# ygjwd12345/UCD

Measured on NVIDIA B200. Metric: ucd_loss_fwd_bwd_pixel_pairs_per_s, higher is better.
Workload: dtype bf16 operands / f32 accumulate (contrastive); f32 (CE, KD, upsample)

## Files before the change

### include/ucd_b200.h

```cpp
#ifndef UCD_B200_H
#define UCD_B200_H

#include <stddef.h>
#include <stdint.h>

#ifdef __cplusplus
extern "C" {
#endif

#define UCD_OK 0
#define UCD_EINVAL (-1)
#define UCD_ECUDA (-2)
#define UCD_ENOSUP (-3)

#define UCD_REDUCTION_NONE 0
#define UCD_REDUCTION_MEAN 1
#define UCD_REDUCTION_SUM 2

#define UCD_FEAT_DIM 256
#define UCD_TILE 128

int ucd_version(void);
const char* ucd_last_error(void);
int ucd_device_ok(void);

int ucd_unce_fwd(const float* x, int64_t* y, float* loss_px, float* lse_all, float* lse_old,
                 float* stats , float* scratch ,
                 int B, int C, int old_cl, int64_t HW, int ignore_index, void* stream);
int ucd_unce_bwd(const float* x, const int64_t* y, const float* lse_all,
                 const float* bkg_gap ,
                 const float* g_px, const float* g_scalar, float g_mul, const float* stats,
                 int mean_over_valid, float* dx, int accumulate, int B, int C, int old_cl, int64_t HW,
                 int ignore_index, void* stream);

int ucd_unkd_fwd(const float* x, const float* t, const float* mask, float alpha, float* out_px,
                 float* stats, float* lse3, float* scratch, int B, int C, int C_old, int64_t HW,
                 void* stream);
int ucd_unkd_bwd(const float* x, const float* t, const float* mask, float alpha, const float* lse3,
                 const float* g_px, const float* g_scalar, float g_mul, float* dx, int accumulate, int B, int C,
                 int C_old, int64_t HW, void* stream);
size_t ucd_reduce_scratch_floats(void);

int ucd_kd_fwd(const float* x, const float* t, const float* mask, float alpha, float* out_px, float* stats,
               float* lse3, float* scratch, int B, int C, int C_old, int64_t HW, int variant, float stats_scale,
               void* stream);
int ucd_kd_bwd(const float* x, const float* t, const float* mask, float alpha, const float* lse3,
               const float* g_px, const float* g_scalar, float g_mul, float* dx, int accumulate, int B, int C,
               int C_old, int64_t HW, int variant, void* stream);
int ucd_unce_unkd_bwd(const float* x, const int64_t* y, const float* lse_all, const float* bkg_gap ,
                      const float* ce_g_px, const float* ce_g_scalar, float ce_g_mul, const float* ce_stats,
                      int mean_over_valid, int old_cl, int ignore_index, const float* t, const float* mask,
                      float alpha, const float* lse3, const float* kd_g_px, const float* kd_g_scalar, float kd_g_mul,
                      int kd_variant, float* dx, int accumulate, int B, int C, int C_old, int64_t HW, void* stream);
int ucd_bkg_mask(const float* t_old, const int64_t* labels, float* mask, int B, int C_old, int64_t HW,
                 int old_cl, void* stream);

int ucd_upsample_bilinear_fwd(const float* in, float* out, int64_t planes, int h, int w, int H, int W,
                              void* stream);
int ucd_upsample_bilinear_bwd(const float* gout, float* gin, int64_t planes, int h, int w, int H, int W,
                              void* stream);

size_t ucd_seg_fused_workspace_floats(int B, int C, int C_old, int h, int w, int H, int W);
int ucd_seg_fused_fwd(const float* lr, const float* lr_old, int64_t* labels, float* g_ce, float* g_kd,
                      float* sums, float* workspace, size_t workspace_floats, int B, int C, int C_old, int h,
                      int w, int H, int W, int old_cl, int ignore_index, float alpha, int need_grad,
                      void* stream);

int64_t ucd_con_max_tiles(int64_t n_px);
int ucd_con_prob_kpad(int C_old);
int ucd_con_num_bins(int max_label, int C_old);
int64_t ucd_con_px_meta_ints(int64_t n_px);
int64_t ucd_con_blk_meta_ints(int64_t n_px, int nb);
int ucd_con_prep_labels(const int64_t* labels, const float* l_po, int B, int C_old, int h, int w,
                        int H, int W, int max_label, int32_t* px_meta, int32_t* blk_meta, int32_t* counts,
                        int32_t* counts_host ,
                        void* stream);
int ucd_con_prep_pack(const float* f_n, const float* f_o, const float* l_po, const int32_t* px_meta,
                      int32_t* blk_meta, const int32_t* counts, int B, int C_old, int h, int w, int max_label,
                      float* anchor_f32, float* contrast_f32, void* la, void* lc,
                      int label_bytes ,
                      void* feat_tiles, void* prob_tiles, int32_t* lab_tiles, int32_t* tile_range,
                      int32_t* row_range , int32_t* row_ref, float* inv_norm,
                      int64_t max_tiles, void* stream);
int ucd_con_prep_bwd(const float* g_anchor, const float* anchor_f32, const float* inv_norm,
                     const int32_t* px_meta, const int32_t* blk_meta, float* df_n, int B, int h, int w,
                     void* stream);
int ucd_con_prep_pack_bf16(const void* f_n, const void* f_o, const float* l_po, const int32_t* px_meta,
                           int32_t* blk_meta, const int32_t* counts, int B, int C_old, int h, int w, int max_label,
                           float* anchor_f32, float* contrast_f32, void* la, void* lc, int label_bytes,
                           void* feat_tiles, void* prob_tiles, int32_t* lab_tiles, int32_t* tile_range,
                           int32_t* row_range, int32_t* row_ref, float* inv_norm, int64_t max_tiles, void* stream);
int ucd_con_prep_bwd_bf16(const float* g_anchor, const float* anchor_f32, const float* inv_norm,
                          const int32_t* px_meta, const int32_t* blk_meta, void* df_n, int B, int h, int w,
                          void* stream);
int ucd_con_tile_ranges(const int32_t* lab_tiles, int64_t n_tiles, const int32_t* n_limit, int32_t* tile_range,
                        void* stream);
int ucd_con_pack_rows(const float* rows, const int32_t* labels, int64_t n, void* feat_tiles,
                      int32_t* lab_tiles, int64_t max_tiles, void* stream);

int ucd_rows_normalize_fwd(const float* f, float* rows, float* inv_norm, int B, int h, int w, void* stream);
int ucd_rows_normalize_bwd(const float* g_rows, const float* rows, const float* inv_norm, float* df, int B, int h,
                           int w, void* stream);

size_t ucd_con_workspace_bytes(int64_t max_row_tiles, int64_t max_col_tiles, int64_t plan_row_tiles,
                               int64_t local_col_tiles );
int ucd_con_fwd(const void* feat_tiles, const void* prob_tiles, const int32_t* lab_tiles,
                const int32_t* chunk_counts, int n_chunks, int64_t chunk_tiles, int64_t chunk_stride_bytes,
                int local_chunk, int part, const void* row_feat_tiles,
                const void* row_prob_tiles, const int32_t* row_lab_tiles, const int32_t* n_rows,
                const int32_t* tile_range, const int32_t* row_range, int64_t self_tile0, const int32_t* min_new, int p_mode, int kpad, const float* dense_p,
                int64_t ldp, float inv_temperature, int need_grad, float* out, float* grad_unit,
                void* workspace, size_t workspace_bytes, int64_t max_row_tiles, int64_t plan_row_tiles,
                void* stream);
size_t ucd_selfcon_workspace_bytes(int64_t tiles );
int ucd_selfcon_fwd(const void* feat_tiles, const int32_t* lab_tiles, const int32_t* tile_range, const int32_t* counts,
                    const int32_t* n_rows, int64_t n, int64_t n_anchor, int mode, float inv_temperature, float kappa,
                    int need_grad, float* out, float* grad_unit, void* workspace, size_t workspace_bytes, void* stream);
int ucd_con_bwd(const float* grad_unit, const float* out, const float* g_scalar, float g_mul,
                const int32_t* n_rows, const int32_t* row_ref, float* d_anchor, int64_t max_rows, void* stream);

#ifdef __cplusplus
}
#endif
#endif
```

### ucd_b200/_lib.py

```python
import ctypes
import os
from ctypes import c_float, c_int, c_int64, c_size_t, c_void_p

_HERE = os.path.dirname(os.path.abspath(__file__))
LIB_PATH = os.path.join(_HERE, "libucd_b200.so")

_lib = None

P = c_void_p
_PROTOS = {
    "ucd_version": (c_int, []),
    "ucd_last_error": (ctypes.c_char_p, []),
    "ucd_device_ok": (c_int, []),
    "ucd_reduce_scratch_floats": (c_size_t, []),
    "ucd_unce_fwd": (c_int, [P, P, P, P, P, P, P, c_int, c_int, c_int, c_int64, c_int, P]),
    "ucd_unce_bwd": (c_int, [P, P, P, P, P, P, c_float, P, c_int, P, c_int, c_int, c_int, c_int, c_int64, c_int, P]),
    "ucd_unkd_fwd": (c_int, [P, P, P, c_float, P, P, P, P, c_int, c_int, c_int, c_int64, P]),
    "ucd_unkd_bwd": (c_int, [P, P, P, c_float, P, P, P, c_float, P, c_int, c_int, c_int, c_int, c_int64, P]),
    "ucd_kd_fwd": (c_int, [P, P, P, c_float, P, P, P, P, c_int, c_int, c_int, c_int64, c_int, c_float, P]),
    "ucd_kd_bwd": (c_int, [P, P, P, c_float, P, P, P, c_float, P, c_int, c_int, c_int, c_int, c_int64, c_int, P]),
    "ucd_unce_unkd_bwd": (c_int, [P, P, P, P, P, P, c_float, P, c_int, c_int, c_int, P, P, c_float, P, P, P, c_float, c_int,
                                  P, c_int, c_int, c_int, c_int, c_int64, P]),
    "ucd_bkg_mask": (c_int, [P, P, P, c_int, c_int, c_int64, c_int, P]),
    "ucd_upsample_bilinear_fwd": (c_int, [P, P, c_int64, c_int, c_int, c_int, c_int, P]),
    "ucd_upsample_bilinear_bwd": (c_int, [P, P, c_int64, c_int, c_int, c_int, c_int, P]),
    "ucd_seg_fused_workspace_floats": (c_size_t, [c_int, c_int, c_int, c_int, c_int, c_int, c_int]),
    "ucd_seg_fused_fwd": (c_int, [P, P, P, P, P, P, P, c_size_t, c_int, c_int, c_int, c_int, c_int, c_int, c_int,
                                  c_int, c_int, c_float, c_int, P]),
    "ucd_con_max_tiles": (c_int64, [c_int64]),
    "ucd_con_prob_kpad": (c_int, [c_int]),
    "ucd_con_num_bins": (c_int, [c_int, c_int]),
    "ucd_con_px_meta_ints": (c_int64, [c_int64]),
    "ucd_con_blk_meta_ints": (c_int64, [c_int64, c_int]),
    "ucd_con_prep_labels": (c_int, [P, P, c_int, c_int, c_int, c_int, c_int, c_int, c_int, P, P, P, P, P]),
    "ucd_con_prep_pack": (c_int, [P, P, P, P, P, P, c_int, c_int, c_int, c_int, c_int, P, P, P, P, c_int, P, P, P, P,
                                  P, P, P, c_int64, P]),
    "ucd_con_prep_bwd": (c_int, [P, P, P, P, P, P, c_int, c_int, c_int, P]),
    "ucd_con_prep_pack_bf16": (c_int, [P, P, P, P, P, P, c_int, c_int, c_int, c_int, c_int, P, P, P, P, c_int, P, P, P,
                                       P, P, P, P, c_int64, P]),
    "ucd_con_prep_bwd_bf16": (c_int, [P, P, P, P, P, P, c_int, c_int, c_int, P]),
    "ucd_rows_normalize_fwd": (c_int, [P, P, P, c_int, c_int, c_int, P]),
    "ucd_rows_normalize_bwd": (c_int, [P, P, P, P, c_int, c_int, c_int, P]),
    "ucd_con_tile_ranges": (c_int, [P, c_int64, P, P, P]),
    "ucd_con_pack_rows": (c_int, [P, P, c_int64, P, P, c_int64, P]),
    "ucd_con_workspace_bytes": (c_size_t, [c_int64, c_int64, c_int64, c_int64]),
    "ucd_con_fwd": (c_int, [P, P, P, P, c_int, c_int64, c_int64, c_int, c_int, P, P, P, P, P, P, c_int64, P, c_int, c_int,
                            P, c_int64, c_float, c_int, P, P, P, c_size_t, c_int64, c_int64, P]),
    "ucd_con_bwd": (c_int, [P, P, P, c_float, P, P, P, c_int64, P]),
    "ucd_selfcon_workspace_bytes": (c_size_t, [c_int64]),
    "ucd_selfcon_fwd": (c_int, [P, P, P, P, P, c_int64, c_int64, c_int, c_float, c_float, c_int, P, P, P, c_size_t, P]),
}
EXPORTED = tuple(_PROTOS)
_DEBUG_PROTOS = {
    "ucd_con_debug_trace": (c_int, [P]),
    "ucd_con_debug_splits": (c_int, [c_int64, c_int64]),
    "ucd_selftest_umma": (c_int, [c_int, ctypes.POINTER(c_float)]),
    "ucd_selftest_mma_rate": (c_int, [c_int, c_int, ctypes.POINTER(c_float)]),
    "ucd_selftest_mma_mix": (c_int, [c_int] * 8 + [ctypes.POINTER(c_float)]),
    "ucd_selftest_pipe_rate": (c_int, [c_int, c_int, c_int, ctypes.POINTER(c_float)]),
    "ucd_selftest_read_probe": (c_int, [P, ctypes.c_longlong, c_int, c_int, c_int, c_int, ctypes.POINTER(c_float)]),
}
DEBUG_EXPORTED = tuple(_DEBUG_PROTOS)
DEBUG_LIB_PATH = os.path.join(_HERE, "libucd_b200_debug.so")
_debug = None


def lib():
    global _lib
    if _lib is None:
        if not os.path.exists(LIB_PATH):
            raise RuntimeError(
                "ucd_b200: %s is missing - build it with `python -m ucd_b200.build` "
                "(there is no CPU or PyTorch fallback for this path)" % LIB_PATH)
        h = ctypes.CDLL(LIB_PATH)
        for name, (res, args) in _PROTOS.items():
            fn = getattr(h, name)
            fn.restype = res
            fn.argtypes = args
        _lib = h
    return _lib


def debug_lib(as_product=False):
    global _debug, _lib
    if _debug is None:
        if not os.path.exists(DEBUG_LIB_PATH):
            raise RuntimeError("ucd_b200: %s is missing - build it with `python -m ucd_b200.build --debug`" % DEBUG_LIB_PATH)
        h = ctypes.CDLL(DEBUG_LIB_PATH)
        for name, (res, args) in list(_PROTOS.items()) + list(_DEBUG_PROTOS.items()):
            fn = getattr(h, name)
            fn.restype = res
            fn.argtypes = args
        _debug = h
    if as_product:
        _lib = _debug
    return _debug


class _NvtxProxy:

    def __init__(self, handle):
        self._h = handle

    def __getattr__(self, name):
        fn = getattr(self._h, name)
        if not name.startswith("ucd_") or name in ("ucd_last_error", "ucd_version", "ucd_device_ok"):
            return fn
        import torch

        def wrapped(*args):
            torch.cuda.nvtx.range_push(name)
            try:
                return fn(*args)
            finally:
                torch.cuda.nvtx.range_pop()
        return wrapped


def enable_nvtx(on=True):
    global _lib
    h = lib()
    if on and not isinstance(h, _NvtxProxy):
        _lib = _NvtxProxy(h)
    elif not on and isinstance(h, _NvtxProxy):
        _lib = h._h


def check(rc, what=""):
    if rc != 0:
        msg = lib().ucd_last_error().decode("utf-8", "replace")
        raise RuntimeError("ucd_b200 %s failed (code %d): %s" % (what, rc, msg))


def ptr(t):
    if t is None:
        return None
    return c_void_p(t) if isinstance(t, int) else c_void_p(t.data_ptr())


_raw_stream = None


def cur_stream():
    global _raw_stream
    import torch
    if _raw_stream is None:
        get_raw = getattr(torch._C, "_cuda_getCurrentRawStream", None)
        get_dev = getattr(torch._C, "_cuda_getDevice", None)
        if get_raw is not None and get_dev is not None:
            _raw_stream = lambda: get_raw(get_dev())
        else:
            _raw_stream = lambda: torch.cuda.current_stream().cuda_stream
    return c_void_p(_raw_stream())
```

### ucd_b200/csrc/ce_kd.cu

```cuda
#include "common.cuh"

namespace ucd {

constexpr int kStreamThreads = 256;
constexpr int kStreamMaxBlocks = kNumSMs * 8;
constexpr int kScratchFloats = 4 * kStreamMaxBlocks + 64;

template <int VEC>
struct Vec;
template <>
struct Vec<4> {
  static __device__ __forceinline__ void load(const float* p, float (&v)[4]) {
    float4 t = ldg_stream4(p);
    v[0] = t.x, v[1] = t.y, v[2] = t.z, v[3] = t.w;
  }
  static __device__ __forceinline__ void load_cached(const float* p, float (&v)[4]) {
    float4 t = *reinterpret_cast<const float4*>(p);
    v[0] = t.x, v[1] = t.y, v[2] = t.z, v[3] = t.w;
  }
  static __device__ __forceinline__ void store(float* p, const float (&v)[4]) {
    *reinterpret_cast<float4*>(p) = make_float4(v[0], v[1], v[2], v[3]);
  }
  static __device__ __forceinline__ void store_stream(float* p, const float (&v)[4]) {
    stg_stream4(p, make_float4(v[0], v[1], v[2], v[3]));
  }
};
template <>
struct Vec<1> {
  static __device__ __forceinline__ void load(const float* p, float (&v)[1]) { v[0] = ldg_stream1(p); }
  static __device__ __forceinline__ void load_cached(const float* p, float (&v)[1]) { v[0] = *p; }
  static __device__ __forceinline__ void store(float* p, const float (&v)[1]) { *p = v[0]; }
  static __device__ __forceinline__ void store_stream(float* p, const float (&v)[1]) { stg_stream1(p, v[0]); }
};

template <int VEC, bool ACC>
__device__ __forceinline__ void store_dx(float* p, float (&o)[VEC]) {
  if (ACC) {
    float old[VEC];
    Vec<VEC>::load(p, old);
#pragma unroll
    for (int i = 0; i < VEC; ++i) o[i] += old[i];
  }
  Vec<VEC>::store_stream(p, o);
}

__global__ void reduce_partials_kernel(const float* __restrict__ part, int nblk, int nk, float* __restrict__ out,
                                       float scale) {
  __shared__ float red[32];
  for (int k = 0; k < nk; ++k) {
    float acc = 0.f;
    for (int i = threadIdx.x; i < nblk; i += blockDim.x) acc += part[(size_t)k * nblk + i];
    float r = block_sum(acc, red);
    if (threadIdx.x == 0) out[k] = r * scale;
  }
}

constexpr float kNegBig = -3.0e38f;
constexpr int kLseChunk = 8;

template <int VEC, bool PICK>
__device__ __forceinline__ void lse_chunks(const float* __restrict__ xp, long long HW, int c0, int c1,
                                           const long long (&lab)[VEC], float (&m)[VEC], float (&s)[VEC],
                                           float (&picked)[VEC]) {
  for (int c = c0; c < c1; c += kLseChunk) {
    float v[kLseChunk][VEC];
#pragma unroll
    for (int k = 0; k < kLseChunk; ++k) {
      if (c + k < c1) {
        Vec<VEC>::load(xp + (long long)(c + k) * HW, v[k]);
      } else {
#pragma unroll
        for (int i = 0; i < VEC; ++i) v[k][i] = kNegBig;
      }
    }
#pragma unroll
    for (int i = 0; i < VEC; ++i) {
      float cm = v[0][i];
#pragma unroll
      for (int k = 1; k < kLseChunk; ++k) cm = fmaxf(cm, v[k][i]);
      const float nm = fmaxf(m[i], cm * kLog2e);
      float acc = s[i] * ex2f(m[i] - nm);
#pragma unroll
      for (int k = 0; k < kLseChunk; ++k) {
        acc += ex2f(fmaf(v[k][i], kLog2e, -nm));
        if (PICK) picked[i] = (lab[i] == c + k) ? v[k][i] : picked[i];
      }
      m[i] = nm;
      s[i] = acc;
    }
  }
}

template <int VEC>
__device__ __forceinline__ void lse_chunk4(const float (&v)[4][VEC], float (&m)[VEC], float (&s)[VEC]) {
#pragma unroll
  for (int i = 0; i < VEC; ++i) {
    const float cm = fmaxf(fmaxf(v[0][i], v[1][i]), fmaxf(v[2][i], v[3][i]));
    const float nm = fmaxf(m[i], cm * kLog2e);
    float acc = s[i] * ex2f(m[i] - nm);
#pragma unroll
    for (int k = 0; k < 4; ++k) acc += ex2f(fmaf(v[k][i], kLog2e, -nm));
    m[i] = nm;
    s[i] = acc;
  }
}

template <int VEC>
__device__ __forceinline__ void lse_planes(const float*& xc, long long HW, int n, float (&m)[VEC], float (&s)[VEC]) {
  int c = 0;
  for (; c + 4 <= n; c += 4) {
    float v[4][VEC];
    Vec<VEC>::load(xc, v[0]);
    Vec<VEC>::load(xc + HW, v[1]);
    Vec<VEC>::load(xc + 2 * HW, v[2]);
    Vec<VEC>::load(xc + 3 * HW, v[3]);
    xc += 4 * HW;
    lse_chunk4<VEC>(v, m, s);
  }
  if (c < n) {
    float v[4][VEC];
#pragma unroll
    for (int k = 0; k < 4; ++k) {
      if (c + k < n) {
        Vec<VEC>::load(xc + k * HW, v[k]);
      } else {
#pragma unroll
        for (int i = 0; i < VEC; ++i) v[k][i] = kNegBig;
      }
    }
    xc += (long long)(n - c) * HW;
    lse_chunk4<VEC>(v, m, s);
  }
}

__device__ __forceinline__ void group_to_bp(long long g, long long gpi, bool small, int vec, long long& b, long long& p) {
  if (small) {
    const unsigned bb = (unsigned)g / (unsigned)gpi;
    b = bb;
    p = (long long)((unsigned)g - bb * (unsigned)gpi) * vec;
  } else {
    b = g / gpi;
    p = (g - b * gpi) * vec;
  }
}

template <int VEC>
__global__ void __launch_bounds__(kStreamThreads, VEC == 4 ? 4 : 2)
unce_fwd_kernel(const float* __restrict__ x, long long* __restrict__ y, float* __restrict__ loss_px,
                float* __restrict__ lse_all_out, float* __restrict__ lse_old_out, float* __restrict__ part,
                int B, int C, int old_cl, long long HW, int ignore_index) {
  const long long gpi = HW / VEC;
  const long long n_groups = gpi * B;
  const bool small = n_groups < (1ll << 31) && gpi < (1ll << 31);
  const int oc = old_cl < C ? (old_cl > 0 ? old_cl : 0) : C;
  float loss_acc = 0.f, valid_acc = 0.f;
  for (long long g = (long long)blockIdx.x * blockDim.x + threadIdx.x; g < n_groups;
       g += (long long)gridDim.x * blockDim.x) {
    long long b, p;
    group_to_bp(g, gpi, small, VEC, b, p);
    const float* xp = x + (b * C) * HW + p;
    long long* yp = y + b * HW + p;
    long long yl[VEC];
    if (VEC == 4) {
      const longlong2 t0 = *reinterpret_cast<const longlong2*>(yp), t1 = *reinterpret_cast<const longlong2*>(yp + 2);
      yl[0] = t0.x, yl[1] = t0.y, yl[2 % VEC] = t1.x, yl[3 % VEC] = t1.y;
    } else {
#pragma unroll
      for (int i = 0; i < VEC; ++i) yl[i] = yp[i];
    }
    int lab[VEC];
    float picked[VEC];
#pragma unroll
    for (int i = 0; i < VEC; ++i) {
      long long t = yl[i];
      if (t < old_cl) {
        if (t != 0) yp[i] = 0;
        t = 0;
      }
      lab[i] = (t < 0 || t > 0x7fffffffLL) ? -1 : (int)t;
      picked[i] = (lab[i] >= 0 && lab[i] < C) ? __ldg(xp + (long long)lab[i] * HW + i) : 0.f;
    }
    float m[VEC], s[VEC], lse_old2[VEC];
#pragma unroll
    for (int i = 0; i < VEC; ++i) m[i] = kNegBig, s[i] = 0.f;
    const float* xc = xp;
    lse_planes<VEC>(xc, HW, oc, m, s);
#pragma unroll
    for (int i = 0; i < VEC; ++i) lse_old2[i] = m[i] + lg2f(s[i]);
    lse_planes<VEC>(xc, HW, C - oc, m, s);
    float out[VEC], la[VEC], lo[VEC];
#pragma unroll
    for (int i = 0; i < VEC; ++i) {
      const float lse2 = m[i] + lg2f(s[i]);
      la[i] = lse2 * kLn2;
      lo[i] = lse_old2[i] * kLn2;
      const bool ign = lab[i] == ignore_index;
      float l = (lab[i] == 0 && old_cl > 0) ? (la[i] - lo[i]) : (la[i] - picked[i]);
      if (ign || lab[i] < 0 || lab[i] >= C) l = 0.f;
      out[i] = l;
      loss_acc += l;
      valid_acc += ign ? 0.f : 1.f;
    }
    Vec<VEC>::store(loss_px + b * HW + p, out);
    Vec<VEC>::store(lse_all_out + b * HW + p, la);
    if (lse_old_out != nullptr) Vec<VEC>::store(lse_old_out + b * HW + p, lo);
  }
  if (part != nullptr) {
    __shared__ float red[32];
    float r0 = block_sum(loss_acc, red);
    float r1 = block_sum(valid_acc, red);
    if (threadIdx.x == 0) {
      part[blockIdx.x] = r0;
      part[gridDim.x + blockIdx.x] = r1;
    }
  }
}

template <int VEC, bool ACC>
__global__ void __launch_bounds__(kStreamThreads)
unce_bwd_kernel(const float* __restrict__ x, const long long* __restrict__ y, const float* __restrict__ lse_all,
                const float* __restrict__ bkg_gap, const float* __restrict__ g_px,
                const float* __restrict__ g_scalar, float g_mul, const float* __restrict__ stats,
                int mean_over_valid, float* __restrict__ dx, int B, int C, int old_cl, long long HW,
                int ignore_index) {
  const long long gpi = HW / VEC;
  const long long n_groups = gpi * B;
  float gs = 0.f;
  if (g_px == nullptr) {
    gs = g_scalar[0] * g_mul;
    if (mean_over_valid) gs = gs / stats[1];
  }
  for (long long g = (long long)blockIdx.x * blockDim.x + threadIdx.x; g < n_groups;
       g += (long long)gridDim.x * blockDim.x) {
    const long long b = g / gpi, p = (g - b * gpi) * VEC;
    const float* xp = x + (b * C) * HW + p;
    float* dp = dx + (b * C) * HW + p;
    const long long* yp = y + b * HW + p;
    float la2[VEC], up[VEC], fold[VEC];
    int lab[VEC];
    {
      float la[VEC], lo[VEC], gp[VEC];
      Vec<VEC>::load_cached(lse_all + b * HW + p, la);
      Vec<VEC>::load_cached(bkg_gap + b * HW + p, lo);
      if (g_px != nullptr) Vec<VEC>::load_cached(g_px + b * HW + p, gp);
#pragma unroll
      for (int i = 0; i < VEC; ++i) {
        long long t = yp[i];
        if (t < old_cl) t = 0;
        const bool dead = (t == ignore_index) || t < 0 || t >= C;
        lab[i] = dead ? -1 : (int)t;
        up[i] = dead ? 0.f : (g_px != nullptr ? gp[i] : gs);
        la2[i] = la[i] * kLog2e;
        fold[i] = ex2f(lo[i] * kLog2e);
      }
    }
#pragma unroll 4
    for (int c = 0; c < C; ++c) {
      float v[VEC], o[VEC];
      Vec<VEC>::load(xp + (long long)c * HW, v);
#pragma unroll
      for (int i = 0; i < VEC; ++i) {
        const float pr = ex2f(fmaf(v[i], kLog2e, -la2[i]));
        float sub;
        if (lab[i] == 0 && old_cl > 0)
          sub = (c < old_cl) ? pr * fold[i] : 0.f;
        else
          sub = (c == lab[i]) ? 1.f : 0.f;
        o[i] = up[i] * (pr - sub);
      }
      store_dx<VEC, ACC>(dp + (long long)c * HW, o);
    }
  }
}

template <int VEC, bool TAIL>
__device__ __forceinline__ void unkd_old_chunk(const float (&v)[4][VEC], const float (&u)[4][VEC], int nv, bool skip0,
                                               float a2, float (&m)[VEC], float (&s)[VEC], float (&mt)[VEC],
                                               float (&st)[VEC], float (&wx)[VEC]) {
#pragma unroll
  for (int i = 0; i < VEC; ++i) {
    float cm = v[0][i], ct = u[0][i] * a2;
#pragma unroll
    for (int k = 1; k < 4; ++k) {
      const bool live = !TAIL || k < nv;
      cm = live ? fmaxf(cm, v[k][i]) : cm;
      ct = live ? fmaxf(ct, u[k][i] * a2) : ct;
    }
    const float nm = fmaxf(m[i], cm * kLog2e), nt = fmaxf(mt[i], ct);
    float acc = s[i] * ex2f(m[i] - nm);
    const float rs = ex2f(mt[i] - nt);
    float tacc = st[i] * rs, wacc = wx[i] * rs;
#pragma unroll
    for (int k = 0; k < 4; ++k) {
      const bool live = !TAIL || k < nv;
      const float ex = ex2f(fmaf(v[k][i], kLog2e, -nm));
      const float et = ex2f(fmaf(u[k][i], a2, -nt));
      acc += live ? ex : 0.f;
      tacc += live ? et : 0.f;
      const float w = (live && !(k == 0 && skip0)) ? et : 0.f;
      wacc = fmaf(w, v[k][i], wacc);
    }
    m[i] = nm, s[i] = acc, mt[i] = nt, st[i] = tacc, wx[i] = wacc;
  }
}

template <int VEC>
__global__ void __launch_bounds__(kStreamThreads, VEC == 4 ? 3 : 2)
unkd_fwd_kernel(const float* __restrict__ x, const float* __restrict__ t, const float* __restrict__ mask,
                float alpha, float* __restrict__ out_px, float* __restrict__ lse3, float* __restrict__ part,
                int B, int C, int Cs, int C_old, int mask_zero, long long HW) {
  const long long gpi = HW / VEC;
  const long long n_groups = gpi * B;
  const bool small = n_groups < (1ll << 31) && gpi < (1ll << 31);
  const long long plane = (long long)B * HW;
  const float a2 = alpha * kLog2e;
  const float inv_cold = 1.f / (float)C_old;
  float acc = 0.f;
  for (long long g = (long long)blockIdx.x * blockDim.x + threadIdx.x; g < n_groups;
       g += (long long)gridDim.x * blockDim.x) {
    long long b, p;
    group_to_bp(g, gpi, small, VEC, b, p);
    const float* xp = x + (b * Cs) * HW + p;
    const float* xc = xp;
    const float* tc = t + (b * C_old) * HW + p;
    float m[VEC], s[VEC], mt[VEC], st[VEC], wx[VEC], x0[VEC], t0[VEC];
#pragma unroll
    for (int i = 0; i < VEC; ++i) m[i] = mt[i] = kNegBig, s[i] = st[i] = wx[i] = 0.f;
    int c = 0;
    for (; c + 4 <= C_old; c += 4) {
      float v[4][VEC], u[4][VEC];
#pragma unroll
      for (int k = 0; k < 4; ++k) {
        Vec<VEC>::load(xc + k * HW, v[k]);
        Vec<VEC>::load(tc + k * HW, u[k]);
      }
      xc += 4 * HW, tc += 4 * HW;
      if (c == 0) {
#pragma unroll
        for (int i = 0; i < VEC; ++i) x0[i] = v[0][i], t0[i] = u[0][i] * a2;
      }
      unkd_old_chunk<VEC, false>(v, u, 4, c == 0, a2, m, s, mt, st, wx);
    }
    if (c < C_old) {
      const int nv = C_old - c;
      float v[4][VEC], u[4][VEC];
#pragma unroll
      for (int k = 0; k < 4; ++k) {
        if (k < nv) {
          Vec<VEC>::load(xc + k * HW, v[k]);
          Vec<VEC>::load(tc + k * HW, u[k]);
        } else {
#pragma unroll
          for (int i = 0; i < VEC; ++i) v[k][i] = 0.f, u[k][i] = 0.f;
        }
      }
      if (c == 0) {
#pragma unroll
        for (int i = 0; i < VEC; ++i) x0[i] = v[0][i], t0[i] = u[0][i] * a2;
      }
      unkd_old_chunk<VEC, true>(v, u, nv, c == 0, a2, m, s, mt, st, wx);
    }
    float mn[VEC], sn[VEC];
#pragma unroll
    for (int i = 0; i < VEC; ++i) mn[i] = kNegBig, sn[i] = 0.f;
    xc = xp + (long long)C_old * HW;
    lse_planes<VEC>(xc, HW, C - C_old, mn, sn);
    float o[VEC], l_all[VEC], l_bkg[VEC], l_t[VEC];
    float mk[VEC];
    if (mask != nullptr) Vec<VEC>::load_cached(mask + b * HW + p, mk);
#pragma unroll
    for (int i = 0; i < VEC; ++i) {
      const float ma = fmaxf(m[i], mn[i]);
      const float lse2 = ma + lg2f(fmaf(s[i], ex2f(m[i] - ma), sn[i] * ex2f(mn[i] - ma)));
      const float x02 = x0[i] * kLog2e;
      const float mb = fmaxf(x02, mn[i]);
      const float lseb2 = mb + lg2f(fmaf(sn[i], ex2f(mn[i] - mb), ex2f(x02 - mb)));
      const float lset2 = mt[i] + lg2f(st[i]);
      l_all[i] = lse2 * kLn2;
      l_bkg[i] = lseb2 * kLn2;
      l_t[i] = lset2 * kLn2;
      const float q0 = ex2f(t0[i] - lset2);
      const float dot = wx[i] / st[i];
      float l = (q0 * (l_bkg[i] - l_all[i]) + dot - (1.f - q0) * l_all[i]) * inv_cold;
      if (mask != nullptr) l *= mask_zero ? (mk[i] == 0.f ? 1.f : 0.f) : mk[i];
      o[i] = -l;
      acc += l;
    }
    if (out_px != nullptr) Vec<VEC>::store(out_px + b * HW + p, o);
    Vec<VEC>::store(lse3 + b * HW + p, l_all);
    Vec<VEC>::store(lse3 + plane + b * HW + p, l_bkg);
    Vec<VEC>::store(lse3 + 2 * plane + b * HW + p, l_t);
  }
  __shared__ float red[32];
  float r = block_sum(acc, red);
  if (threadIdx.x == 0) part[blockIdx.x] = r;
}

template <int VEC, bool ACC>
__global__ void __launch_bounds__(kStreamThreads)
unkd_bwd_kernel(const float* __restrict__ x, const float* __restrict__ t, const float* __restrict__ mask,
                float alpha, const float* __restrict__ lse3, const float* __restrict__ g_px,
                const float* __restrict__ g_scalar, float g_mul, float* __restrict__ dx, int B, int C, int Cs,
                int C_old, int mask_zero, long long HW) {
  const long long gpi = HW / VEC;
  const long long n_groups = gpi * B;
  const long long plane = (long long)B * HW;
  const float a2 = alpha * kLog2e;
  const float inv_cold = 1.f / (float)C_old;
  const float gs = (g_px == nullptr) ? g_scalar[0] * g_mul : 0.f;
  for (long long g = (long long)blockIdx.x * blockDim.x + threadIdx.x; g < n_groups;
       g += (long long)gridDim.x * blockDim.x) {
    const long long b = g / gpi, p = (g - b * gpi) * VEC;
    const float* xp = x + (b * Cs) * HW + p;
    const float* tp = t + (b * C_old) * HW + p;
    float* dp = dx + (b * Cs) * HW + p;
    float la2[VEC], lt2[VEC], up[VEC], fb[VEC];
    {
      float la[VEC], lb[VEC], lt[VEC], gp[VEC], mk[VEC], u0[VEC];
      Vec<VEC>::load_cached(lse3 + b * HW + p, la);
      Vec<VEC>::load_cached(lse3 + plane + b * HW + p, lb);
      Vec<VEC>::load_cached(lse3 + 2 * plane + b * HW + p, lt);
      Vec<VEC>::load_cached(tp, u0);
      if (g_px != nullptr) Vec<VEC>::load_cached(g_px + b * HW + p, gp);
      if (mask != nullptr) Vec<VEC>::load_cached(mask + b * HW + p, mk);
#pragma unroll
      for (int i = 0; i < VEC; ++i) {
        la2[i] = la[i] * kLog2e;
        lt2[i] = lt[i] * kLog2e;
        float u = (g_px != nullptr ? gp[i] : gs) * inv_cold;
        if (mask != nullptr) u *= mask_zero ? (mk[i] == 0.f ? 1.f : 0.f) : mk[i];
        up[i] = u;
        const float q0 = ex2f(fmaf(u0[i], a2, -lt2[i]));
        fb[i] = q0 * ex2f((la[i] - lb[i]) * kLog2e);
      }
    }
    {
      float v[VEC], o[VEC];
      Vec<VEC>::load(xp, v);
#pragma unroll
      for (int i = 0; i < VEC; ++i) {
        const float pr = ex2f(fmaf(v[i], kLog2e, -la2[i]));
        o[i] = up[i] * (pr - pr * fb[i]);
      }
      store_dx<VEC, ACC>(dp, o);
    }
#pragma unroll 4
    for (int c = 1; c < C_old; ++c) {
      float v[VEC], u[VEC], o[VEC];
      Vec<VEC>::load(xp + (long long)c * HW, v);
      Vec<VEC>::load(tp + (long long)c * HW, u);
#pragma unroll
      for (int i = 0; i < VEC; ++i) {
        const float pr = ex2f(fmaf(v[i], kLog2e, -la2[i]));
        const float q = ex2f(fmaf(u[i], a2, -lt2[i]));
        o[i] = up[i] * (pr - q);
      }
      store_dx<VEC, ACC>(dp + (long long)c * HW, o);
    }
#pragma unroll 4
    for (int c = C_old; c < C; ++c) {
      float v[VEC], o[VEC];
      Vec<VEC>::load(xp + (long long)c * HW, v);
#pragma unroll
      for (int i = 0; i < VEC; ++i) {
        const float pr = ex2f(fmaf(v[i], kLog2e, -la2[i]));
        o[i] = up[i] * (pr - pr * fb[i]);
      }
      store_dx<VEC, ACC>(dp + (long long)c * HW, o);
    }
    if (!ACC)
      for (int c = C; c < Cs; ++c) {
        float o[VEC];
#pragma unroll
        for (int i = 0; i < VEC; ++i) o[i] = 0.f;
        Vec<VEC>::store_stream(dp + (long long)c * HW, o);
      }
  }
}

template <int VEC, bool ACC>
__global__ void __launch_bounds__(kStreamThreads)
unce_unkd_bwd_kernel(const float* __restrict__ x, const long long* __restrict__ y, const float* __restrict__ lse_all,
                     const float* __restrict__ bkg_gap, const float* __restrict__ ce_g_px,
                     const float* __restrict__ ce_g_scalar, float ce_g_mul, const float* __restrict__ ce_stats,
                     int mean_over_valid, int old_cl, int ignore_index, const float* __restrict__ t,
                     const float* __restrict__ mask, float alpha, const float* __restrict__ lse3,
                     const float* __restrict__ kd_g_px, const float* __restrict__ kd_g_scalar, float kd_g_mul,
                     int mask_zero, float* __restrict__ dx, int B, int C, int C_old, long long HW) {
  const long long gpi = HW / VEC;
  const long long n_groups = gpi * B;
  const long long plane = (long long)B * HW;
  const float a2 = alpha * kLog2e;
  const float inv_cold = 1.f / (float)C_old;
  float gs_ce = 0.f;
  if (ce_g_px == nullptr) {
    gs_ce = ce_g_scalar[0] * ce_g_mul;
    if (mean_over_valid) gs_ce = gs_ce / ce_stats[1];
  }
  const float gs_kd = (kd_g_px == nullptr) ? kd_g_scalar[0] * kd_g_mul : 0.f;
  for (long long g = (long long)blockIdx.x * blockDim.x + threadIdx.x; g < n_groups;
       g += (long long)gridDim.x * blockDim.x) {
    const long long b = g / gpi, p = (g - b * gpi) * VEC;
    const float* xp = x + (b * C) * HW + p;
    const float* tp = t + (b * C_old) * HW + p;
    float* dp = dx + (b * C) * HW + p;
    const long long* yp = y + b * HW + p;
    float la2[VEC], lt2[VEC], uce[VEC], ukd[VEC], fold[VEC], fb[VEC];
    int lab[VEC];
    {
      float la[VEC], lo[VEC], lb[VEC], lt[VEC], gp[VEC], gk[VEC], mk[VEC], u0[VEC];
      Vec<VEC>::load_cached(lse_all + b * HW + p, la);
      Vec<VEC>::load_cached(bkg_gap + b * HW + p, lo);
      Vec<VEC>::load_cached(lse3 + plane + b * HW + p, lb);
      Vec<VEC>::load_cached(lse3 + 2 * plane + b * HW + p, lt);
      Vec<VEC>::load_cached(tp, u0);
      if (ce_g_px != nullptr) Vec<VEC>::load_cached(ce_g_px + b * HW + p, gp);
      if (kd_g_px != nullptr) Vec<VEC>::load_cached(kd_g_px + b * HW + p, gk);
      if (mask != nullptr) Vec<VEC>::load_cached(mask + b * HW + p, mk);
#pragma unroll
      for (int i = 0; i < VEC; ++i) {
        long long tt = yp[i];
        if (tt < old_cl) tt = 0;
        const bool dead = (tt == ignore_index) || tt < 0 || tt >= C;
        lab[i] = dead ? -1 : (int)tt;
        uce[i] = dead ? 0.f : (ce_g_px != nullptr ? gp[i] : gs_ce);
        la2[i] = la[i] * kLog2e;
        lt2[i] = lt[i] * kLog2e;
        fold[i] = ex2f(lo[i] * kLog2e);
        float u = (kd_g_px != nullptr ? gk[i] : gs_kd) * inv_cold;
        if (mask != nullptr) u *= mask_zero ? (mk[i] == 0.f ? 1.f : 0.f) : mk[i];
        ukd[i] = u;
        const float q0 = ex2f(fmaf(u0[i], a2, -lt2[i]));
        fb[i] = q0 * ex2f((la[i] - lb[i]) * kLog2e);
      }
    }
#pragma unroll 4
    for (int c = 0; c < C; ++c) {
      float v[VEC], u[VEC], o[VEC];
      Vec<VEC>::load(xp + (long long)c * HW, v);
      const bool old_fg = c >= 1 && c < C_old;
      if (old_fg) Vec<VEC>::load(tp + (long long)c * HW, u);
#pragma unroll
      for (int i = 0; i < VEC; ++i) {
        const float pr = ex2f(fmaf(v[i], kLog2e, -la2[i]));
        float sub_ce;
        if (lab[i] == 0 && old_cl > 0)
          sub_ce = (c < old_cl) ? pr * fold[i] : 0.f;
        else
          sub_ce = (c == lab[i]) ? 1.f : 0.f;
        const float sub_kd = old_fg ? ex2f(fmaf(u[i], a2, -lt2[i])) : pr * fb[i];
        o[i] = fmaf(uce[i], pr - sub_ce, ukd[i] * (pr - sub_kd));
      }
      store_dx<VEC, ACC>(dp + (long long)c * HW, o);
    }
  }
}

__global__ void __launch_bounds__(kStreamThreads)
bkg_mask_kernel(const float* __restrict__ t, const long long* __restrict__ y, float* __restrict__ mask, int B,
                int C_old, long long HW, int old_cl) {
  const long long n = (long long)B * HW;
  for (long long g = (long long)blockIdx.x * blockDim.x + threadIdx.x; g < n; g += (long long)gridDim.x * blockDim.x) {
    const long long b = g / HW, p = g - b * HW;
    const float* tp = t + (b * C_old) * HW + p;
    const float t0 = ldg_stream1(tp);
    const bool t0_nan = t0 != t0;
    bool bkg = true;
    for (int c = 1; c < C_old; ++c) {
      const float v = ldg_stream1(tp + (long long)c * HW);
      if (!t0_nan && (v > t0 || v != v)) bkg = false;
    }
    mask[g] = (bkg || y[g] > old_cl) ? 1.f : 0.f;
  }
}

static int stream_grid(long long n_groups) {
  long long blocks = (n_groups + kStreamThreads - 1) / kStreamThreads;
  if (blocks > kStreamMaxBlocks) blocks = kStreamMaxBlocks;
  if (blocks < 1) blocks = 1;
  return (int)blocks;
}

static bool can_vec4(long long HW, std::initializer_list<const void*> ptrs) {
  if (HW % 4 != 0) return false;
  for (const void* p : ptrs)
    if (p != nullptr && !aligned16(p)) return false;
  return true;
}

}

using namespace ucd;

extern "C" size_t ucd_reduce_scratch_floats(void) { return (size_t)kScratchFloats; }

extern "C" int ucd_unce_fwd(const float* x, int64_t* y, float* loss_px, float* lse_all, float* lse_old,
                            float* stats, float* scratch, int B, int C, int old_cl, int64_t HW,
                            int ignore_index, void* stream) {
  UCD_CHECK_ARG(x && y && loss_px && lse_all, "ucd_unce_fwd: null pointer");
  UCD_CHECK_ARG(B > 0 && C > 0 && HW > 0, "ucd_unce_fwd: bad shape B=%d C=%d HW=%lld", B, C, (long long)HW);
  UCD_CHECK_ARG(old_cl >= 0 && old_cl <= C, "ucd_unce_fwd: old_cl=%d outside [0,%d]", old_cl, C);
  UCD_CHECK_ARG(stats == nullptr || scratch != nullptr, "ucd_unce_fwd: stats requested without scratch");
  cudaStream_t st = (cudaStream_t)stream;
  float* part = stats ? scratch : nullptr;
  const bool v4 = can_vec4(HW, {x, loss_px, lse_all, lse_old}) && aligned16(y);
  const int grid = stream_grid((long long)B * HW / (v4 ? 4 : 1));
  if (v4)
    unce_fwd_kernel<4><<<grid, kStreamThreads, 0, st>>>(x, (long long*)y, loss_px, lse_all, lse_old, part, B, C,
                                                        old_cl, HW, ignore_index);
  else
    unce_fwd_kernel<1><<<grid, kStreamThreads, 0, st>>>(x, (long long*)y, loss_px, lse_all, lse_old, part, B, C,
                                                        old_cl, HW, ignore_index);
  UCD_CHECK_LAUNCH("unce_fwd_kernel");
  if (stats) {
    reduce_partials_kernel<<<1, 256, 0, st>>>(part, grid, 2, stats, 1.f);
    UCD_CHECK_LAUNCH("reduce_partials_kernel");
  }
  return UCD_OK;
}

extern "C" int ucd_unce_bwd(const float* x, const int64_t* y, const float* lse_all, const float* bkg_gap,
                            const float* g_px, const float* g_scalar, float g_mul, const float* stats,
                            int mean_over_valid, float* dx, int accumulate, int B, int C, int old_cl, int64_t HW,
                            int ignore_index, void* stream) {
  UCD_CHECK_ARG(x && y && lse_all && bkg_gap && dx, "ucd_unce_bwd: null pointer");
  UCD_CHECK_ARG(g_px || g_scalar, "ucd_unce_bwd: need g_px or g_scalar");
  UCD_CHECK_ARG(!mean_over_valid || stats, "ucd_unce_bwd: mean_over_valid needs stats");
  UCD_CHECK_ARG(B > 0 && C > 0 && HW > 0, "ucd_unce_bwd: bad shape");
  cudaStream_t st = (cudaStream_t)stream;
  const bool v4 = can_vec4(HW, {x, lse_all, bkg_gap, g_px, dx}) && aligned16(y);
  const int grid = stream_grid((long long)B * HW / (v4 ? 4 : 1));
  auto kern = v4 ? (accumulate ? unce_bwd_kernel<4, true> : unce_bwd_kernel<4, false>)
                 : (accumulate ? unce_bwd_kernel<1, true> : unce_bwd_kernel<1, false>);
  kern<<<grid, kStreamThreads, 0, st>>>(x, (const long long*)y, lse_all, bkg_gap, g_px, g_scalar, g_mul, stats,
                                        mean_over_valid, dx, B, C, old_cl, HW, ignore_index);
  UCD_CHECK_LAUNCH("unce_bwd_kernel");
  return UCD_OK;
}

static int kd_fwd_impl(const float* x, const float* t, const float* mask, float alpha, float* out_px, float* stats,
                       float* lse3, float* scratch, int B, int C, int C_old, int64_t HW, int variant, float stats_scale,
                       void* stream) {
  UCD_CHECK_ARG(x && t && stats && lse3 && scratch, "ucd_kd_fwd: null pointer");
  UCD_CHECK_ARG(B > 0 && HW > 0 && C_old >= 1 && C >= C_old, "ucd_kd_fwd: bad shape C=%d C_old=%d", C, C_old);
  UCD_CHECK_ARG(variant >= 0 && variant <= 2, "ucd_kd_fwd: bad variant %d", variant);
  cudaStream_t st = (cudaStream_t)stream;
  const int Cu = variant == 1 ? C_old : C, mz = variant == 2 ? 1 : 0;
  const bool v4 = can_vec4(HW, {x, t, mask, out_px, lse3}) && ((long long)B * HW) % 4 == 0;
  const int grid = stream_grid((long long)B * HW / (v4 ? 4 : 1));
  if (v4)
    unkd_fwd_kernel<4><<<grid, kStreamThreads, 0, st>>>(x, t, mask, alpha, out_px, lse3, scratch, B, Cu, C, C_old, mz, HW);
  else
    unkd_fwd_kernel<1><<<grid, kStreamThreads, 0, st>>>(x, t, mask, alpha, out_px, lse3, scratch, B, Cu, C, C_old, mz, HW);
  UCD_CHECK_LAUNCH("unkd_fwd_kernel");
  reduce_partials_kernel<<<1, 256, 0, st>>>(scratch, grid, 1, stats, stats_scale);
  UCD_CHECK_LAUNCH("reduce_partials_kernel");
  return UCD_OK;
}

static int kd_bwd_impl(const float* x, const float* t, const float* mask, float alpha, const float* lse3,
                       const float* g_px, const float* g_scalar, float g_mul, float* dx, int accumulate, int B, int C,
                       int C_old, int64_t HW, int variant, void* stream) {
  UCD_CHECK_ARG(x && t && lse3 && dx, "ucd_kd_bwd: null pointer");
  UCD_CHECK_ARG(g_px || g_scalar, "ucd_kd_bwd: need g_px or g_scalar");
  UCD_CHECK_ARG(B > 0 && HW > 0 && C_old >= 1 && C >= C_old, "ucd_kd_bwd: bad shape");
  UCD_CHECK_ARG(variant >= 0 && variant <= 2, "ucd_kd_bwd: bad variant %d", variant);
  cudaStream_t st = (cudaStream_t)stream;
  const int Cu = variant == 1 ? C_old : C, mz = variant == 2 ? 1 : 0;
  const bool v4 = can_vec4(HW, {x, t, mask, g_px, lse3, dx}) && ((long long)B * HW) % 4 == 0;
  const int grid = stream_grid((long long)B * HW / (v4 ? 4 : 1));
  auto kern = v4 ? (accumulate ? unkd_bwd_kernel<4, true> : unkd_bwd_kernel<4, false>)
                 : (accumulate ? unkd_bwd_kernel<1, true> : unkd_bwd_kernel<1, false>);
  kern<<<grid, kStreamThreads, 0, st>>>(x, t, mask, alpha, lse3, g_px, g_scalar, g_mul, dx, B, Cu, C, C_old, mz, HW);
  UCD_CHECK_LAUNCH("unkd_bwd_kernel");
  return UCD_OK;
}

extern "C" int ucd_unkd_fwd(const float* x, const float* t, const float* mask, float alpha, float* out_px,
                            float* stats, float* lse3, float* scratch, int B, int C, int C_old, int64_t HW,
                            void* stream) {
  return kd_fwd_impl(x, t, mask, alpha, out_px, stats, lse3, scratch, B, C, C_old, HW, 0, 1.f, stream);
}

extern "C" int ucd_unkd_bwd(const float* x, const float* t, const float* mask, float alpha, const float* lse3,
                            const float* g_px, const float* g_scalar, float g_mul, float* dx, int accumulate, int B,
                            int C, int C_old, int64_t HW, void* stream) {
  return kd_bwd_impl(x, t, mask, alpha, lse3, g_px, g_scalar, g_mul, dx, accumulate, B, C, C_old, HW, 0, stream);
}

extern "C" int ucd_kd_fwd(const float* x, const float* t, const float* mask, float alpha, float* out_px,
                          float* stats, float* lse3, float* scratch, int B, int C, int C_old, int64_t HW,
                          int variant, float stats_scale, void* stream) {
  return kd_fwd_impl(x, t, mask, alpha, out_px, stats, lse3, scratch, B, C, C_old, HW, variant, stats_scale, stream);
}

extern "C" int ucd_kd_bwd(const float* x, const float* t, const float* mask, float alpha, const float* lse3,
                          const float* g_px, const float* g_scalar, float g_mul, float* dx, int accumulate, int B,
                          int C, int C_old, int64_t HW, int variant, void* stream) {
  return kd_bwd_impl(x, t, mask, alpha, lse3, g_px, g_scalar, g_mul, dx, accumulate, B, C, C_old, HW, variant, stream);
}

extern "C" int ucd_bkg_mask(const float* t_old, const int64_t* labels, float* mask, int B, int C_old, int64_t HW,
                            int old_cl, void* stream) {
  UCD_CHECK_ARG(t_old && labels && mask, "ucd_bkg_mask: null pointer");
  UCD_CHECK_ARG(B > 0 && C_old >= 1 && HW > 0, "ucd_bkg_mask: bad shape");
  bkg_mask_kernel<<<stream_grid((long long)B * HW), kStreamThreads, 0, (cudaStream_t)stream>>>(
      t_old, (const long long*)labels, mask, B, C_old, HW, old_cl);
  UCD_CHECK_LAUNCH("bkg_mask_kernel");
  return UCD_OK;
}

extern "C" int ucd_unce_unkd_bwd(const float* x, const int64_t* y, const float* lse_all, const float* bkg_gap,
                                 const float* ce_g_px, const float* ce_g_scalar, float ce_g_mul, const float* ce_stats,
                                 int mean_over_valid, int old_cl, int ignore_index, const float* t, const float* mask,
                                 float alpha, const float* lse3, const float* kd_g_px, const float* kd_g_scalar,
                                 float kd_g_mul, int kd_variant, float* dx, int accumulate, int B, int C, int C_old,
                                 int64_t HW, void* stream) {
  UCD_CHECK_ARG(x && y && lse_all && bkg_gap && t && lse3 && dx, "ucd_unce_unkd_bwd: null pointer");
  UCD_CHECK_ARG((ce_g_px || ce_g_scalar) && (kd_g_px || kd_g_scalar), "ucd_unce_unkd_bwd: need g_px or g_scalar for both terms");
  UCD_CHECK_ARG(!mean_over_valid || ce_stats, "ucd_unce_unkd_bwd: mean_over_valid needs stats");
  UCD_CHECK_ARG(B > 0 && HW > 0 && C_old >= 1 && C >= C_old, "ucd_unce_unkd_bwd: bad shape");
  UCD_CHECK_ARG(kd_variant == 0 || kd_variant == 2, "ucd_unce_unkd_bwd: KD variant must be 0 (unbiased) or 2 (masked)");
  cudaStream_t st = (cudaStream_t)stream;
  const bool v4 = can_vec4(HW, {x, lse_all, bkg_gap, ce_g_px, t, mask, lse3, kd_g_px, dx}) && aligned16(y) &&
                  ((long long)B * HW) % 4 == 0;
  const int grid = stream_grid((long long)B * HW / (v4 ? 4 : 1));
  auto kern = v4 ? (accumulate ? unce_unkd_bwd_kernel<4, true> : unce_unkd_bwd_kernel<4, false>)
                 : (accumulate ? unce_unkd_bwd_kernel<1, true> : unce_unkd_bwd_kernel<1, false>);
  kern<<<grid, kStreamThreads, 0, st>>>(x, (const long long*)y, lse_all, bkg_gap, ce_g_px, ce_g_scalar, ce_g_mul,
                                        ce_stats, mean_over_valid, old_cl, ignore_index, t, mask, alpha, lse3, kd_g_px,
                                        kd_g_scalar, kd_g_mul, kd_variant == 2 ? 1 : 0, dx, B, C, C_old, HW);
  UCD_CHECK_LAUNCH("unce_unkd_bwd_kernel");
  return UCD_OK;
}
```

### ucd_b200/csrc/upsample.cu

```cuda
#include "common.cuh"

#include <stdlib.h>

namespace ucd {

constexpr int kUpThreads = 256;

template <int VEC>
__global__ void __launch_bounds__(kUpThreads)
upsample_fwd_kernel(const float* __restrict__ in, float* __restrict__ out, long long planes, int h, int w, int H,
                    int W, float scale_h, float scale_w, int planes_per_block) {
  const int wv = (W + VEC - 1) / VEC;
  const long long idx = (long long)blockIdx.x * blockDim.x + threadIdx.x;
  if (idx >= (long long)H * wv) return;
  const int Y = (int)(idx / wv);
  const int X = (int)(idx - (long long)Y * wv) * VEC;
  const Tap ty = bilinear_tap(Y, scale_h, h, H);
  int x0[VEC], x1[VEC];
  float wx0[VEC], wx1[VEC];
  const bool small_out = H + W <= 128;
  bool uniform = true;
#pragma unroll
  for (int i = 0; i < VEC; ++i) {
    const Tap tx = bilinear_tap(X + i, scale_w, w, W);
    x0[i] = tx.i0, x1[i] = tx.i1, wx0[i] = tx.w0, wx1[i] = tx.w1;
    uniform = uniform && tx.i0 == x0[0] && tx.i1 == x1[0];
  }
  const long long p0 = (long long)blockIdx.y * planes_per_block;
  const long long p1 = (p0 + planes_per_block < planes) ? p0 + planes_per_block : planes;
  const size_t in_plane = (size_t)h * w, out_plane = (size_t)H * W;
  float* dst = out + p0 * out_plane + (size_t)Y * W + X;
  if (uniform) {
    const float* s00 = in + p0 * in_plane + ty.i0 * w + x0[0];
    const int d01 = x1[0] - x0[0], d10 = (ty.i1 - ty.i0) * w;
    constexpr int UP = 4;
    long long p = p0;
    for (; p + UP <= p1; p += UP) {
      float v[UP][4];
#pragma unroll
      for (int u = 0; u < UP; ++u) {
        const float* s = s00 + u * in_plane;
        v[u][0] = __ldg(s), v[u][1] = __ldg(s + d01), v[u][2] = __ldg(s + d10), v[u][3] = __ldg(s + d10 + d01);
      }
#pragma unroll
      for (int u = 0; u < UP; ++u) {
        float r[VEC];
#pragma unroll
        for (int i = 0; i < VEC; ++i)
          r[i] = bilinear_blend(small_out, v[u][0], v[u][1], v[u][2], v[u][3], ty.w0, ty.w1, wx0[i], wx1[i]);
        if (VEC == 4)
          stg_stream4(dst + u * out_plane, make_float4(r[0], r[1], r[2], r[3]));
        else
          stg_stream1(dst + u * out_plane, r[0]);
      }
      s00 += UP * in_plane;
      dst += UP * out_plane;
    }
    for (; p < p1; ++p) {
      const float a = __ldg(s00), b = __ldg(s00 + d01), c = __ldg(s00 + d10), d = __ldg(s00 + d10 + d01);
      float r[VEC];
#pragma unroll
      for (int i = 0; i < VEC; ++i) r[i] = bilinear_blend(small_out, a, b, c, d, ty.w0, ty.w1, wx0[i], wx1[i]);
      if (VEC == 4)
        stg_stream4(dst, make_float4(r[0], r[1], r[2], r[3]));
      else
        stg_stream1(dst, r[0]);
      s00 += in_plane;
      dst += out_plane;
    }
    return;
  }
  for (long long p = p0; p < p1; ++p) {
    const float* src = in + p * in_plane;
    float r[VEC];
#pragma unroll
    for (int i = 0; i < VEC; ++i)
      r[i] = bilinear_blend(small_out, __ldg(src + ty.i0 * w + x0[i]), __ldg(src + ty.i0 * w + x1[i]),
                            __ldg(src + ty.i1 * w + x0[i]), __ldg(src + ty.i1 * w + x1[i]), ty.w0, ty.w1, wx0[i],
                            wx1[i]);
    if (VEC == 4)
      stg_stream4(dst, make_float4(r[0], r[1], r[2], r[3]));
    else
      stg_stream1(dst, r[0]);
    dst += out_plane;
  }
}

constexpr int kUpMaxIvRows = 96;
template <int VEC>
__global__ void __launch_bounds__(kUpThreads)
upsample_fwd_interval_kernel(const float* __restrict__ in, float* __restrict__ out, int h, int w, int H, int W,
                             float scale_h, float scale_w, int tw, int n_col_tiles) {
  __shared__ float s_h0[kUpMaxIvRows], s_h1[kUpMaxIvRows];
  __shared__ int s_lo[3], s_hi[3];
  const int wv = (W + VEC - 1) / VEC;
  const int rp = kUpThreads / tw;
  const int per_plane = h * n_col_tiles;
  const long long plane = blockIdx.x / per_plane;
  const int rem = (int)(blockIdx.x - plane * per_plane);
  const int k = rem / n_col_tiles, col_tile = rem - k * n_col_tiles;
  const float inv = (float)H / (float)h;
  int lo = (int)floorf(((float)k - 0.5f) * inv) - 2, hi = (int)ceilf(((float)k + 1.5f) * inv) + 2;
  lo = max(lo, 0), hi = min(hi, H - 1);
  if (threadIdx.x < kUpMaxIvRows) {
    const int Y = lo + (int)threadIdx.x;
    bool match = false;
    if (Y <= hi) {
      const Tap ty = bilinear_tap(Y, scale_h, h, H);
      match = ty.i0 == k;
      s_h0[threadIdx.x] = ty.w0, s_h1[threadIdx.x] = ty.w1;
    }
    const unsigned bal = __ballot_sync(0xffffffffu, match);
    if ((threadIdx.x & 31) == 0) {
      const int wq = threadIdx.x >> 5;
      s_lo[wq] = bal ? wq * 32 + __ffs(bal) - 1 : 1 << 30;
      s_hi[wq] = bal ? wq * 32 + 31 - __clz(bal) : -1;
    }
  }
  __syncthreads();
  const int ia = min(s_lo[0], min(s_lo[1], s_lo[2])), ib = max(s_hi[0], max(s_hi[1], s_hi[2]));
  const int nrow = ib - ia + 1;
  if (nrow <= 0) return;
  const int Ya = lo + ia;
  const int xg = col_tile * tw + (int)threadIdx.x % tw, rphase = (int)threadIdx.x / tw;
  if (xg >= wv || rphase >= rp) return;
  const int X = xg * VEC;
  const int k1 = min(k + 1, h - 1);
  const float* r0 = in + (size_t)plane * h * w + (size_t)k * w;
  const float* r1 = in + (size_t)plane * h * w + (size_t)k1 * w;
  float t0[VEC], t1[VEC];
#pragma unroll
  for (int i = 0; i < VEC; ++i) {
    const Tap tx = bilinear_tap(min(X + i, W - 1), scale_w, w, W);
    t0[i] = __fmaf_rn(__ldg(r0 + tx.i0), tx.w0, __fmul_rn(__ldg(r0 + tx.i1), tx.w1));
    t1[i] = __fmaf_rn(__ldg(r1 + tx.i0), tx.w0, __fmul_rn(__ldg(r1 + tx.i1), tx.w1));
  }
  float* dst = out + (size_t)plane * H * W + (size_t)(Ya + rphase) * W + X;
  const size_t step = (size_t)rp * W;
#pragma unroll 4
  for (int r = rphase; r < nrow; r += rp) {
    const float h0 = s_h0[ia + r], h1 = s_h1[ia + r];
    float o[VEC];
#pragma unroll
    for (int i = 0; i < VEC; ++i) o[i] = __fmaf_rn(t0[i], h0, __fmul_rn(t1[i], h1));
    if (VEC == 4)
      stg_stream4(dst, make_float4(o[0], o[1], o[2], o[3]));
    else
      stg_stream1(dst, o[0]);
    dst += step;
  }
}

template <int RY, int VEC>
__global__ void __launch_bounds__(kUpThreads)
upsample_bwd_kernel(const float* __restrict__ gout, float* __restrict__ gin, int h, int w, int H, int W,
                    float scale_h, float scale_w, float inv_scale_h, float inv_scale_w, int ny_cap) {
  extern __shared__ __align__(16) float up_smem[];
  float* colsum = up_smem;
  float* wrow = up_smem + (size_t)RY * W;
  const long long plane = blockIdx.y;
  const int ybase = blockIdx.x * RY;
  const int ylast = min(ybase + RY, h) - 1;
  const float* g = gout + (size_t)plane * H * W;
  int Ylo = (int)floorf(((float)ybase - 0.5f) * inv_scale_h - 0.5f) - 2;
  int Yhi = (int)ceilf(((float)ylast + 1.5f) * inv_scale_h - 0.5f) + 2;
  Ylo = max(Ylo, 0);
  Yhi = min(Yhi, H - 1);
  if (h == H) {
    Ylo = ybase;
    Yhi = ylast;
  }
  Yhi = min(Yhi, Ylo + ny_cap - 1);
  const int ny = Yhi - Ylo + 1;
  for (int i = threadIdx.x; i < ny; i += kUpThreads) {
    const Tap ty = bilinear_tap(Ylo + i, scale_h, h, H);
#pragma unroll
    for (int r = 0; r < RY; ++r) {
      float wgt = 0.f;
      if (ty.i0 - ybase == r) wgt += ty.w0;
      if (ty.i1 - ybase == r) wgt += ty.w1;
      wrow[i * RY + r] = wgt;
    }
  }
  for (int i = threadIdx.x; i < RY * W; i += kUpThreads) colsum[i] = 0.f;
  __syncthreads();
  const int ngroups = (W + VEC - 1) / VEC;
  const int nsplit = max(1, min(kUpThreads / ngroups, 8));
  const int team = threadIdx.x / ngroups;
  const bool working = team < nsplit || ngroups >= kUpThreads;
  for (int g0 = 0; g0 < ngroups; g0 += kUpThreads) {
    const int xg = g0 + (ngroups >= kUpThreads ? threadIdx.x : threadIdx.x - team * ngroups);
    float acc[RY][VEC];
#pragma unroll
    for (int r = 0; r < RY; ++r)
#pragma unroll
      for (int k = 0; k < VEC; ++k) acc[r][k] = 0.f;
    if (working && xg < ngroups) {
      const int ystep = ngroups >= kUpThreads ? 1 : nsplit;
      const float* gp = g + (size_t)Ylo * W + (size_t)xg * VEC;
#pragma unroll 4
      for (int i = (ngroups >= kUpThreads ? 0 : team); i < ny; i += ystep) {
        float v[VEC];
        if (VEC == 4) {
          const float4 t = ldg_stream4(gp + (size_t)i * W);
          v[0] = t.x, v[1] = t.y, v[2] = t.z, v[3] = t.w;
        } else {
          v[0] = ldg_stream1(gp + (size_t)i * W);
        }
        float wr[RY];
        if (RY == 4) {
          const float4 t = *reinterpret_cast<const float4*>(wrow + i * RY);
          wr[0] = t.x, wr[1] = t.y, wr[2] = t.z, wr[3] = t.w;
        } else {
#pragma unroll
          for (int r = 0; r < RY; ++r) wr[r] = wrow[i * RY + r];
        }
#pragma unroll
        for (int r = 0; r < RY; ++r)
#pragma unroll
          for (int k = 0; k < VEC; ++k) acc[r][k] = fmaf(wr[r], v[k], acc[r][k]);
      }
    }
    for (int s = 0; s < (ngroups >= kUpThreads ? 1 : nsplit); ++s) {
      if (working && xg < ngroups && (ngroups >= kUpThreads || team == s)) {
#pragma unroll
        for (int r = 0; r < RY; ++r)
#pragma unroll
          for (int k = 0; k < VEC; ++k) colsum[r * W + xg * VEC + k] += acc[r][k];
      }
      __syncthreads();
    }
  }
  const int n_out = RY * w;
  for (int o = threadIdx.x; o < n_out; o += kUpThreads) {
    const int r = o / w, x = o - r * w;
    if (ybase + r >= h) continue;
    int Xlo = (int)floorf(((float)x - 0.5f) * inv_scale_w - 0.5f) - 2;
    int Xhi = (int)ceilf(((float)x + 1.5f) * inv_scale_w - 0.5f) + 2;
    Xlo = max(Xlo, 0);
    Xhi = min(Xhi, W - 1);
    if (w == W) Xlo = Xhi = x;
    float acc = 0.f;
    for (int X = Xlo; X <= Xhi; ++X) {
      const Tap tx = bilinear_tap(X, scale_w, w, W);
      float wgt = 0.f;
      if (tx.i0 == x) wgt += tx.w0;
      if (tx.i1 == x) wgt += tx.w1;
      acc = fmaf(wgt, colsum[r * W + X], acc);
    }
    gin[((size_t)plane * h + ybase + r) * w + x] = acc;
  }
}

template <int UN>
__global__ void __launch_bounds__(256, 4)
upsample_bwd_sweep_kernel(const float* __restrict__ gout, float* __restrict__ gin, int h, int w, int H, int W,
                          float scale_h, float scale_w, long long total_rows, int cap_rows, int ny_cap) {
  extern __shared__ __align__(16) uint8_t up_dyn[];
  const int wv = blockDim.x;
  const int tid = threadIdx.x;
  float4* ring = reinterpret_cast<float4*>(up_dyn);
  float2* s_p = reinterpret_cast<float2*>(ring + (size_t)UN * wv);
  float2* s_h = s_p + 2 * wv;
  int* s_k = reinterpret_cast<int*>(s_h + ny_cap);
  int* s_x0 = s_k + ny_cap;
  int* s_x1 = s_x0 + wv;
  short4* s_j = reinterpret_cast<short4*>(s_x1 + wv);
  __shared__ int s_lim[2];
  const int X = tid * 4;
  float wx0[4], wx1[4];
  {
    const Tap t0 = bilinear_tap(X, scale_w, w, W);
    s_x0[tid] = t0.i0, s_x1[tid] = t0.i1;
#pragma unroll
    for (int i = 0; i < 4; ++i) {
      const Tap tx = bilinear_tap(X + i, scale_w, w, W);
      wx0[i] = tx.w0, wx1[i] = tx.w1;
    }
  }
  __syncthreads();
  if (tid < w) {
    const int sc4 = (W / w) / 4;
    const int j0 = max((tid - 2) * sc4 - 2, 0), j1 = min((tid + 2) * sc4 + 2, wv - 1);
    int a0 = 0, a1 = 0, b0 = 0, b1 = 0;
    bool fa = false, fb = false;
    for (int j = j0; j <= j1; ++j) {
      if (s_x0[j] == tid) {
        if (!fa) a0 = j, fa = true;
        a1 = j + 1;
      }
      if (s_x1[j] == tid) {
        if (!fb) b0 = j, fb = true;
        b1 = j + 1;
      }
    }
    s_j[tid] = make_short4((short)a0, (short)a1, (short)b0, (short)b1);
  }
  const float inv = (float)H / (float)h;
  const uint32_t ring_s = (uint32_t)__cvta_generic_to_shared(ring + tid);
  const uint32_t slot_b = (uint32_t)wv * 16u;
  int flip = 0;
  const long long r_begin = total_rows * (long long)blockIdx.x / (long long)gridDim.x;
  const long long r_end = total_rows * ((long long)blockIdx.x + 1) / (long long)gridDim.x;
  for (long long r = r_begin; r < r_end;) {
    const long long plane = r / h;
    const int y0 = (int)(r - plane * h);
    const int ylast = (int)min((long long)min(h, y0 + cap_rows), y0 + (r_end - r)) - 1;
    r += ylast - y0 + 1;
    int Ylo = (int)floorf(((float)y0 - 0.5f) * inv) - 2, Yhi = (int)ceilf(((float)ylast + 1.5f) * inv) + 2;
    Ylo = max(Ylo, 0), Yhi = min(Yhi, H - 1);
    const int ny = min(Yhi - Ylo + 1, ny_cap);
    __syncthreads();
    for (int i = tid; i < ny; i += wv) {
      const Tap ty = bilinear_tap(Ylo + i, scale_h, h, H);
      s_k[i] = ty.i0;
      const bool clamped = ty.i1 == ty.i0;
      s_h[i] = make_float2(clamped ? ty.w0 + ty.w1 : ty.w0, clamped ? 0.f : ty.w1);
    }
    __syncthreads();
    for (int i = tid; i < ny; i += wv) {
      const int k = s_k[i];
      if (k >= y0 && k <= ylast) {
        if (i == 0 || s_k[i - 1] < y0) s_lim[0] = i;
        if (i == ny - 1 || s_k[i + 1] > ylast) s_lim[1] = i + 1;
      }
    }
    __syncthreads();
    const int i_lo = s_lim[0], i_hi = s_lim[1];
    const float* gp = gout + (size_t)plane * H * W + (size_t)(Ylo + i_lo) * W + X;
    float* out = gin + (size_t)plane * h * w;
    float a0p0 = 0.f, a0p1 = 0.f, a1p0 = 0.f, a1p1 = 0.f, c0 = 0.f, c1 = 0.f;
    int cur = -1;
    auto emit = [&](int row, float v0, float v1, bool shared) {
      s_p[flip * wv + tid] = make_float2(v0, v1);
      __syncthreads();
      if (tid < w) {
        const short4 jr = s_j[tid];
        const float2* sp = s_p + flip * wv;
        float acc = 0.f;
        for (int j = jr.x; j < jr.y; ++j) acc += sp[j].x;
        for (int j = jr.z; j < jr.w; ++j) acc += sp[j].y;
        if (shared)
          atomicAdd(out + (size_t)row * w + tid, acc);
        else
          out[(size_t)row * w + tid] = acc;
      }
      flip ^= 1;
    };
    auto flush = [&]() {
      emit(cur, a0p0 + c0, a0p1 + c1, cur == y0 && y0 > 0);
      c0 = a1p0, c1 = a1p1;
      a0p0 = a0p1 = a1p0 = a1p1 = 0.f;
    };
    int nfetch = i_hi - i_lo;
    uint32_t fslot = 0, cslot = 0;
    auto fetch = [&]() {
      if (nfetch > 0) {
        asm volatile("cp.async.cg.shared.global [%0], [%1], 16;" ::"r"(ring_s + fslot), "l"(gp) : "memory");
        gp += W;
        --nfetch;
      }
      cp_async_commit();
      fslot = (fslot + slot_b == slot_b * UN) ? 0u : fslot + slot_b;
    };
#pragma unroll
    for (int j = 0; j < UN - 1; ++j) fetch();
#pragma unroll 1
    for (int i = i_lo; i < i_hi; ++i) {
      fetch();
      cp_async_wait<UN - 1>();
      const int k = s_k[i];
      if (k != cur) {
        if (cur >= 0) flush();
        cur = k;
      }
      float4 x;
      asm volatile("ld.shared.v4.f32 {%0,%1,%2,%3}, [%4];" : "=f"(x.x), "=f"(x.y), "=f"(x.z), "=f"(x.w) : "r"(ring_s + cslot));
      cslot = (cslot + slot_b == slot_b * UN) ? 0u : cslot + slot_b;
      const float2 hw = s_h[i];
      const float p0 = fmaf(x.w, wx0[3], fmaf(x.z, wx0[2], fmaf(x.y, wx0[1], x.x * wx0[0])));
      const float p1 = fmaf(x.w, wx1[3], fmaf(x.z, wx1[2], fmaf(x.y, wx1[1], x.x * wx1[0])));
      a0p0 = fmaf(hw.x, p0, a0p0), a0p1 = fmaf(hw.x, p1, a0p1);
      a1p0 = fmaf(hw.y, p0, a1p0), a1p1 = fmaf(hw.y, p1, a1p1);
    }
    cp_async_wait<0>();
    if (cur >= 0) {
      flush();
      if (ylast < h - 1) emit(ylast + 1, c0, c1, true);
    }
  }
}

}

using namespace ucd;

extern "C" int ucd_upsample_bilinear_fwd(const float* in, float* out, int64_t planes, int h, int w, int H, int W,
                                         void* stream) {
  UCD_CHECK_ARG(in && out, "ucd_upsample_bilinear_fwd: null pointer");
  UCD_CHECK_ARG(planes > 0 && h > 0 && w > 0 && H > 0 && W > 0, "ucd_upsample_bilinear_fwd: bad shape");
  UCD_CHECK_ARG((long long)h * w < (1ll << 30), "ucd_upsample_bilinear_fwd: source plane too large");
  cudaStream_t st = (cudaStream_t)stream;
  const float sh = (float)h / (float)H, sw = (float)w / (float)W;
  const bool v4 = (W % 4 == 0) && aligned16(out);
  const int wv = v4 ? W / 4 : W;
  if (H + W > 128 && H >= h && W >= w && (double)H / h <= 40.0  && planes * (long long)h < (1ll << 30) / 64) {
    const int tw = wv < kUpThreads ? wv : kUpThreads;
    const int nct = (wv + tw - 1) / tw;
    const unsigned nblk = (unsigned)(planes * h * nct);
    if (v4)
      upsample_fwd_interval_kernel<4><<<nblk, kUpThreads, 0, st>>>(in, out, h, w, H, W, sh, sw, tw, nct);
    else
      upsample_fwd_interval_kernel<1><<<nblk, kUpThreads, 0, st>>>(in, out, h, w, H, W, sh, sw, tw, nct);
    UCD_CHECK_LAUNCH("upsample_fwd_interval_kernel");
    return UCD_OK;
  }
  const long long work = (long long)H * wv;
  const int gx = (int)((work + kUpThreads - 1) / kUpThreads);
  long long want_y = (32ll * kNumSMs + gx - 1) / gx;
  if (want_y < 1) want_y = 1;
  if (want_y > (planes + 15) / 16) want_y = (planes + 15) / 16;
#ifdef UCD_DEBUG_KNOBS
  if (const char* e = getenv("UCD_UP_GY")) want_y = atoi(e) > 0 ? atoi(e) : want_y;
#endif
  if (want_y > planes) want_y = planes;
  const int ppb = (int)((planes + want_y - 1) / want_y);
  const int gy = (int)((planes + ppb - 1) / ppb);
  UCD_CHECK_ARG(gy <= 65535, "ucd_upsample_bilinear_fwd: too many planes");
  dim3 grid(gx, gy);
  if (v4)
    upsample_fwd_kernel<4><<<grid, kUpThreads, 0, st>>>(in, out, planes, h, w, H, W, sh, sw, ppb);
  else
    upsample_fwd_kernel<1><<<grid, kUpThreads, 0, st>>>(in, out, planes, h, w, H, W, sh, sw, ppb);
  UCD_CHECK_LAUNCH("upsample_fwd_kernel");
  return UCD_OK;
}

extern "C" int ucd_upsample_bilinear_bwd(const float* gout, float* gin, int64_t planes, int h, int w, int H, int W,
                                         void* stream) {
  UCD_CHECK_ARG(gout && gin, "ucd_upsample_bilinear_bwd: null pointer");
  UCD_CHECK_ARG(planes > 0 && h > 0 && w > 0 && H > 0 && W > 0, "ucd_upsample_bilinear_bwd: bad shape");
  cudaStream_t st = (cudaStream_t)stream;
  constexpr int RY = 4;
  const int ny_cap = (h == H) ? RY : (int)((double)(RY + 2) * H / h) + 8;
  const size_t smem = ((size_t)RY * W + (size_t)ny_cap * RY) * sizeof(float);
  UCD_CHECK_ARG(smem <= 200 * 1024, "ucd_upsample_bilinear_bwd: W=%d / scale too large for one block", W);
  const float sh = (float)h / (float)H, sw = (float)w / (float)W;
  const bool v4 = (W % 4 == 0) && aligned16(gout);
  const int up = H / (h > 0 ? h : 1);
  constexpr int kUpSweepTaps = 640;
  const int cap_rows = up > 0 ? (kUpSweepTaps - 8) / up - 2 : 0;
  if (v4 && H % h == 0 && W % w == 0 && (W / w) % 8 == 0 && W / 4 <= 256 && (W / 4) % 32 == 0 && w <= W / 4 &&
      cap_rows >= 1) {
    int un = 8, bps = (W / 4 <= 128 ? 4 : 2);
#ifdef UCD_DEBUG_KNOBS
    if (const char* e = getenv("UCD_UPB_UN")) un = atoi(e);
    if (const char* e = getenv("UCD_UPB_BPS")) bps = atoi(e);
#endif
    const long long total_rows = planes * h;
    long long nb = (long long)kNumSMs * bps;
    while (nb > kNumSMs && total_rows / nb < 4) nb -= kNumSMs;
    if (nb > total_rows) nb = total_rows;
    long long seg = (total_rows + nb - 1) / nb + 1;
    if (seg > cap_rows) seg = cap_rows;
    const int ny_cap = (int)(seg + 2) * up + 8;
    const int wv4 = W / 4;
    const size_t dyn = (size_t)un * wv4 * 16 + (size_t)2 * wv4 * 8 + (size_t)ny_cap * 12 + (size_t)2 * wv4 * 4 + (size_t)w * 8;
    cudaError_t e = cudaMemsetAsync(gin, 0, (size_t)planes * h * w * sizeof(float), st);
    if (e != cudaSuccess) return cuda_fail(e, "cudaMemsetAsync(upsample_bwd)");
    auto kern = upsample_bwd_sweep_kernel<8>;
#ifdef UCD_DEBUG_KNOBS
    if (un == 4) kern = upsample_bwd_sweep_kernel<4>;
    if (un == 12) kern = upsample_bwd_sweep_kernel<12>;
    if (un == 16) kern = upsample_bwd_sweep_kernel<16>;
#endif
    if (dyn > 48 * 1024) {
      e = cudaFuncSetAttribute(kern, cudaFuncAttributeMaxDynamicSharedMemorySize, (int)dyn);
      if (e != cudaSuccess) return cuda_fail(e, "cudaFuncSetAttribute(upsample_bwd_sweep)");
    }
    kern<<<(unsigned)nb, wv4, dyn, st>>>(gout, gin, h, w, H, W, sh, sw, total_rows, cap_rows, ny_cap);
    UCD_CHECK_LAUNCH("upsample_bwd_sweep_kernel");
    return UCD_OK;
  }
  auto kern = v4 ? upsample_bwd_kernel<RY, 4> : upsample_bwd_kernel<RY, 1>;
  if (smem > 48 * 1024) {
    cudaError_t e = cudaFuncSetAttribute(kern, cudaFuncAttributeMaxDynamicSharedMemorySize, (int)smem);
    if (e != cudaSuccess) return cuda_fail(e, "cudaFuncSetAttribute(upsample_bwd)");
  }
  const int gyb = (h + RY - 1) / RY;
  for (int64_t p0 = 0; p0 < planes; p0 += 65535) {
    const int np = (int)((planes - p0 < 65535) ? planes - p0 : 65535);
    dim3 grid(gyb, np);
    kern<<<grid, kUpThreads, smem, st>>>(gout + (size_t)p0 * H * W, gin + (size_t)p0 * h * w, h, w, H, W, sh, sw,
                                         (float)H / (float)h, (float)W / (float)w, ny_cap);
    UCD_CHECK_LAUNCH("upsample_bwd_kernel");
  }
  return UCD_OK;
}
```

### ucd_b200/losses.py

```python
from __future__ import annotations

import torch
import torch.nn as nn

from . import _lib
from ._lib import check, cur_stream, ptr

FEAT_DIM = 256
TILE = 128


def _need_cuda(*tensors):
    cur = None
    for t in tensors:
        if t is None:
            continue
        if not t.is_cuda:
            raise RuntimeError("ucd_b200: expected CUDA tensors (there is no CPU fallback for this path)")
        if cur is None:
            cur = torch.cuda.current_device()
        if t.device.index != cur:
            raise RuntimeError("ucd_b200: tensor on cuda:%d but the current device is cuda:%d - wrap the call in "
                               "`with torch.cuda.device(tensor.device):`" % (t.device.index, cur))


def _f32c(t):
    if t.dtype != torch.float32:
        t = t.float()
    return t.contiguous()


def _scalar_grad(g):
    if g.dim() == 0:
        return g.reshape(1)
    if all(s == 0 for s in g.stride()):
        return g.as_strided((1,), (1,))
    return None


class _UpsampleFn(torch.autograd.Function):
    @staticmethod
    def forward(ctx, x, out_h, out_w):
        _need_cuda(x)
        x = _f32c(x)
        lead, (h, w) = x.shape[:-2], x.shape[-2:]
        planes = 1
        for d in lead:
            planes *= d
        out = torch.empty(*lead, out_h, out_w, device=x.device, dtype=torch.float32)
        if planes > 0:
            check(_lib.lib().ucd_upsample_bilinear_fwd(ptr(x), ptr(out), planes, h, w, out_h, out_w, cur_stream()),
                  "upsample_bilinear_fwd")
        ctx.shape = (lead, h, w, out_h, out_w, planes)
        return out

    @staticmethod
    def backward(ctx, g):
        lead, h, w, out_h, out_w, planes = ctx.shape
        g = _f32c(g)
        gin = torch.empty(*lead, h, w, device=g.device, dtype=torch.float32)
        if planes > 0:
            check(_lib.lib().ucd_upsample_bilinear_bwd(ptr(g), ptr(gin), planes, h, w, out_h, out_w, cur_stream()),
                  "upsample_bilinear_bwd")
        return gin, None, None


def interpolate_bilinear(x, size):
    return _UpsampleFn.apply(x, int(size[0]), int(size[1]))


class _GradChain:

    __slots__ = ("token", "calls", "pending", "closed")
    MAX_MEMBERS = 4

    def __init__(self):
        self.token, self.calls, self.pending, self.closed = None, 0, [], False

    @staticmethod
    def of(t):
        if not (torch.is_grad_enabled() and t.requires_grad and t.dtype == torch.float32 and t.is_contiguous()):
            return None
        chain = getattr(t, "_ucd_grad_chain", None)
        if chain is None or chain.closed or chain.calls >= _GradChain.MAX_MEMBERS:
            chain = t._ucd_grad_chain = _GradChain()
        return chain

    def submit(self, term, seq, is_head):
        self.closed = True
        if seq == self.calls:
            self.pending = []
        if not is_head:
            if term is not None:
                self.pending.append(term)
            return None, None
        terms, self.pending = self.pending + ([term] if term is not None else []), []
        self.token = None
        return (_launch_terms(terms) if terms else None), None


def _launch_terms(terms):
    dx = torch.empty_like(terms[0]["x"])
    ce = [t for t in terms if t["kind"] == "ce"]
    kd = [t for t in terms if t["kind"] == "kd" and t["variant"] in (0, 2)]
    acc = False
    if ce and kd and ce[0]["C"] == kd[0]["C"] and ce[0]["HW"] == kd[0]["HW"]:
        c, k = ce[0], kd[0]
        check(_lib.lib().ucd_unce_unkd_bwd(
            ptr(c["x"]), ptr(c["targets"]), ptr(c["lse"][0]), ptr(c["lse"][1]), ptr(c["g_px"]), ptr(c["g_sc"]), 1.0,
            ptr(c["stats"]), c["mean_over_valid"], c["old_cl"], c["ignore_index"], ptr(k["t"]), ptr(k["m"]), k["alpha"],
            ptr(k["lse3"]), ptr(k["g_px"]), ptr(k["g_sc"]), k["g_mul"], k["variant"], ptr(dx), 0, c["B"], c["C"],
            k["C_old"], c["HW"], cur_stream()), "unce_unkd_bwd")
        terms = [t for t in terms if t is not c and t is not k]
        acc = True
    for t in terms:
        _launch_term(t, dx, acc)
        acc = True
    return dx


def _launch_term(t, dx, acc):
    if t["kind"] == "ce":
        check(_lib.lib().ucd_unce_bwd(ptr(t["x"]), ptr(t["targets"]), ptr(t["lse"][0]), ptr(t["lse"][1]), ptr(t["g_px"]),
                                      ptr(t["g_sc"]), 1.0, ptr(t["stats"]), t["mean_over_valid"], ptr(dx),
                                      1 if acc else 0, t["B"], t["C"], t["old_cl"], t["HW"], t["ignore_index"],
                                      cur_stream()), "unce_bwd")
    else:
        check(_lib.lib().ucd_kd_bwd(ptr(t["x"]), ptr(t["t"]), ptr(t["m"]), t["alpha"], ptr(t["lse3"]), ptr(t["g_px"]),
                                    ptr(t["g_sc"]), t["g_mul"], ptr(dx), 1 if acc else 0, t["B"], t["C"], t["C_old"],
                                    t["HW"], t["variant"], cur_stream()), "kd_bwd")


class _UnceFn(torch.autograd.Function):
    @staticmethod
    def forward(ctx, inputs, targets, old_cl, ignore_index, reduction, chain=None, link=None):
        ctx.chain, ctx.is_head, ctx.seq = chain, link is None, (chain.calls if chain is not None else 0)
        ctx.set_materialize_grads(False)
        B, C = inputs.shape[0], inputs.shape[1]
        HW = inputs.numel() // max(B * C, 1)
        x = _f32c(inputs)
        dev = x.device
        loss_px = torch.empty(targets.shape, device=dev, dtype=torch.float32)
        lse = torch.empty(targets.shape, device=dev, dtype=torch.float32)
        want_stats = reduction != "none"
        stats = torch.empty(2, device=dev, dtype=torch.float32) if want_stats else None
        scratch = (torch.empty(_lib.lib().ucd_reduce_scratch_floats(), device=dev, dtype=torch.float32)
                   if want_stats else None)
        check(_lib.lib().ucd_unce_fwd(ptr(x), ptr(targets), ptr(loss_px), ptr(lse), None, ptr(stats),
                                      ptr(scratch), B, C, old_cl, HW, ignore_index, cur_stream()), "unce_fwd")
        ctx.save_for_backward(x, targets, lse, stats, loss_px)
        ctx.cfg = (B, C, HW, old_cl, ignore_index, reduction)
        out = loss_px if reduction == "none" else (stats[0].clone() if reduction == "sum" else stats[0] / stats[1])
        if chain is None:
            return out
        return out, torch.empty((), device=dev, dtype=torch.float32)

    @staticmethod
    def backward(ctx, g, g_token=None):
        x, targets, lse, stats, loss_px = ctx.saved_tensors
        B, C, HW, old_cl, ignore_index, reduction = ctx.cfg
        if g is None:
            if ctx.chain is None:
                return None, None, None, None, None, None, None
            d_in, d_link = ctx.chain.submit(None, ctx.seq, ctx.is_head)
            return d_in, None, None, None, None, None, d_link
        g_px, g_sc = None, None
        if reduction == "none":
            g_sc = _scalar_grad(g)
            if g_sc is None:
                g_px = _f32c(g)
        else:
            g_sc = g.reshape(1)
        if g_sc is not None:
            g_sc = _f32c(g_sc)
        term = dict(kind="ce", x=x, targets=targets, lse=(lse, loss_px), stats=stats, g_px=g_px, g_sc=g_sc,
                    mean_over_valid=1 if reduction == "mean" else 0, B=B, C=C, HW=HW, old_cl=old_cl,
                    ignore_index=ignore_index)
        if ctx.chain is None:
            dx = torch.empty_like(x)
            _launch_term(term, dx, False)
            return dx, None, None, None, None, None, None
        d_in, d_link = ctx.chain.submit(term, ctx.seq, ctx.is_head)
        return d_in, None, None, None, None, None, d_link


def _chained(fn, inputs, args):
    chain = _GradChain.of(inputs)
    if chain is None:
        return fn.apply(inputs, *args)
    chain.calls += 1
    out, token = fn.apply(inputs, *args, chain, chain.token)
    chain.token = token
    return out


class UnbiasedCrossEntropy(nn.Module):

    def __init__(self, old_cl=None, reduction='mean', ignore_index=255):
        super().__init__()
        self.reduction = reduction
        self.ignore_index = ignore_index
        self.old_cl = old_cl

    def forward(self, inputs, targets):
        _need_cuda(inputs, targets)
        if self.reduction not in ("none", "mean", "sum"):
            raise ValueError("reduction must be 'none', 'mean' or 'sum'")
        if targets.dtype != torch.int64:
            raise TypeError("UnbiasedCrossEntropy: targets must be int64 (train.py:98 casts labels to long)")
        if inputs.dim() < 2 or targets.shape != inputs.shape[:1] + inputs.shape[2:]:
            raise ValueError("UnbiasedCrossEntropy: inputs [B,C,...] and targets [B,...] shapes disagree")
        old_cl = inputs.shape[1] if self.old_cl is None else int(self.old_cl)
        tgt = targets if targets.is_contiguous() else targets.contiguous()
        out = _chained(_UnceFn, inputs, (tgt, old_cl, int(self.ignore_index), self.reduction))
        if tgt is not targets:
            targets.copy_(tgt)
        return out


class _UnkdFn(torch.autograd.Function):
    @staticmethod
    def forward(ctx, inputs, targets, mask, alpha, reduction, variant=0, chain=None, link=None):
        ctx.chain, ctx.is_head, ctx.seq = chain, link is None, (chain.calls if chain is not None else 0)
        ctx.set_materialize_grads(False)
        B, C, C_old = inputs.shape[0], inputs.shape[1], targets.shape[1]
        HW = inputs.numel() // max(B * C, 1)
        x, t = _f32c(inputs), _f32c(targets)
        m = None if mask is None else _f32c(mask)
        dev = x.device
        px_shape = (B,) + tuple(inputs.shape[2:])
        out_px = torch.empty(px_shape, device=dev, dtype=torch.float32) if reduction == "none" else None
        stats = torch.empty(1, device=dev, dtype=torch.float32)
        lse3 = torch.empty((3,) + px_shape, device=dev, dtype=torch.float32)
        scratch = torch.empty(_lib.lib().ucd_reduce_scratch_floats(), device=dev, dtype=torch.float32)
        scale = -1.0 / float(B * HW) if reduction == "mean" else -1.0
        check(_lib.lib().ucd_kd_fwd(ptr(x), ptr(t), ptr(m), float(alpha), ptr(out_px), ptr(stats), ptr(lse3),
                                    ptr(scratch), B, C, C_old, HW, variant, scale, cur_stream()), "kd_fwd")
        ctx.save_for_backward(x, t, m, lse3)
        ctx.cfg = (B, C, C_old, HW, float(alpha), reduction, variant)
        out = out_px if reduction == "none" else stats[0]
        if chain is None:
            return out
        return out, torch.empty((), device=dev, dtype=torch.float32)

    @staticmethod
    def backward(ctx, g, g_token=None):
        x, t, m, lse3 = ctx.saved_tensors
        B, C, C_old, HW, alpha, reduction, variant = ctx.cfg
        if g is None:
            if ctx.chain is None:
                return None, None, None, None, None, None, None, None
            d_in, d_link = ctx.chain.submit(None, ctx.seq, ctx.is_head)
            return d_in, None, None, None, None, None, None, d_link
        g_px, g_sc, g_mul = None, None, 1.0
        if reduction == "none":
            g_sc = _scalar_grad(g)
            if g_sc is None:
                g_px = _f32c(g)
        else:
            g_sc = g.reshape(1)
            if reduction == "mean":
                g_mul = 1.0 / float(B * HW)
        if g_sc is not None:
            g_sc = _f32c(g_sc)
        term = dict(kind="kd", x=x, t=t, m=m, lse3=lse3, g_px=g_px, g_sc=g_sc, g_mul=g_mul, alpha=alpha, B=B, C=C,
                    C_old=C_old, HW=HW, variant=variant)
        if ctx.chain is None:
            dx = torch.empty_like(x)
            _launch_term(term, dx, False)
            return dx, None, None, None, None, None, None, None
        d_in, d_link = ctx.chain.submit(term, ctx.seq, ctx.is_head)
        return d_in, None, None, None, None, None, None, d_link


class UnbiasedKnowledgeDistillationLoss(nn.Module):

    def __init__(self, reduction='mean', alpha=1.):
        super().__init__()
        self.reduction = reduction
        self.alpha = alpha

    def forward(self, inputs, targets, mask=None):
        _need_cuda(inputs, targets, mask)
        if inputs.shape[1] < targets.shape[1] or inputs.shape[2:] != targets.shape[2:]:
            raise ValueError("UnbiasedKnowledgeDistillationLoss: inputs [B,C,...] / targets [B,C_old,...] disagree")
        if mask is not None and tuple(mask.shape) != (inputs.shape[0],) + tuple(inputs.shape[2:]):
            raise ValueError("UnbiasedKnowledgeDistillationLoss: mask must be [B,...]")
        red = self.reduction if self.reduction in ("mean", "sum") else "none"
        return _chained(_UnkdFn, inputs, (targets.detach(), mask, self.alpha, red, 0))


def _kd_forward(name, variant, self, inputs, targets, mask):
    _need_cuda(inputs, targets, mask)
    if inputs.shape[1] < targets.shape[1] or inputs.shape[2:] != targets.shape[2:]:
        raise ValueError("%s: inputs [B,C,...] / targets [B,C_old,...] disagree" % name)
    if mask is not None and tuple(mask.shape) != (inputs.shape[0],) + tuple(inputs.shape[2:]):
        raise ValueError("%s: mask must be [B,...]" % name)
    red = self.reduction if self.reduction in ("mean", "sum") else "none"
    return _chained(_UnkdFn, inputs, (targets.detach(), mask, self.alpha, red, variant))


class KnowledgeDistillationLoss(nn.Module):

    def __init__(self, reduction='mean', alpha=1.):
        super().__init__()
        self.reduction = reduction
        self.alpha = alpha

    def forward(self, inputs, targets, mask=None):
        return _kd_forward("KnowledgeDistillationLoss", 1, self, inputs, targets, mask)


class MaskKnowledgeDistillationLoss(nn.Module):

    def __init__(self, reduction='mean', alpha=1.):
        super().__init__()
        self.reduction = reduction
        self.alpha = alpha

    def forward(self, inputs, targets, mask=None):
        return _kd_forward("MaskKnowledgeDistillationLoss", 2, self, inputs, targets, mask)


class MaskCrossEntropy(nn.Module):

    def __init__(self, old_cl=None, reduction='mean', ignore_index=255):
        super().__init__()
        self.reduction = reduction
        self.ignore_index = ignore_index
        self.old_cl = old_cl

    def forward(self, inputs, targets, outputs_old=None):
        _need_cuda(inputs, targets, outputs_old)
        if targets.dtype != torch.int64:
            raise TypeError("MaskCrossEntropy: targets must be int64")
        if inputs.dim() < 2 or targets.shape != inputs.shape[:1] + inputs.shape[2:]:
            raise ValueError("MaskCrossEntropy: inputs [B,C,...] and targets [B,...] shapes disagree")
        if outputs_old is not None and self.old_cl is None:
            raise TypeError("MaskCrossEntropy: old_cl=None cannot be compared with the labels (loss.py:210)")
        old_cl = 0 if self.old_cl is None else int(self.old_cl)
        ign = int(self.ignore_index)
        if old_cl > 1:
            tgt = torch.where((targets >= 1) & (targets < old_cl), torch.full_like(targets, ign), targets).contiguous()
        else:
            tgt = targets.clone()
        loss = _UnceFn.apply(inputs, tgt, old_cl, ign, "none")
        if outputs_old is not None:
            t = _f32c(outputs_old.detach())
            B, C_old = t.shape[0], t.shape[1]
            mask = torch.empty(targets.shape, device=t.device, dtype=torch.float32)
            lab = targets if targets.is_contiguous() else targets.contiguous()
            check(_lib.lib().ucd_bkg_mask(ptr(t), ptr(lab), ptr(mask), B, C_old, t[0, 0].numel(), old_cl,
                                          cur_stream()), "bkg_mask")
            loss = loss * mask
        if self.reduction == 'mean':
            return -torch.mean(loss)
        if self.reduction == 'sum':
            return -torch.sum(loss)
        return loss


def payload_layout(max_tiles, kpad):
    al = lambda n: (n + 255) & ~255
    off = {"counts": 0}
    o = 256
    for name, nbytes in (("range", max_tiles * 8), ("lab", max_tiles * TILE * 4), ("prob", max_tiles * kpad * TILE * 2),
                         ("feat", max_tiles * FEAT_DIM * TILE * 2)):
        off[name] = o
        o += al(nbytes)
    off["nbytes"] = o
    return off


def payload_views(buf, max_tiles, kpad):
    lay = payload_layout(max_tiles, kpad)
    assert buf.dtype == torch.uint8 and buf.shape[-1] == lay["nbytes"]

    def sec(name, nbytes, dtype, shape):
        v = buf[..., lay[name]:lay[name] + nbytes].view(dtype)
        return v.unflatten(-1, shape)
    T = max_tiles
    return dict(counts=sec("counts", 16, torch.int32, (4,)), range=sec("range", T * 8, torch.int32, (T, 2)),
                lab=sec("lab", T * TILE * 4, torch.int32, (T, TILE)),
                prob=sec("prob", T * kpad * TILE * 2, torch.bfloat16, (T, kpad // 8, TILE, 8)),
                feat=sec("feat", T * FEAT_DIM * TILE * 2, torch.bfloat16, (T, FEAT_DIM // 8, TILE, 8)))


class ContrastPack:

    def __init__(self):
        self.n_px = 0
        self.shape = None
        self.c_old = 0
        self.kpad = 0
        self.max_tiles = 0
        self.payload = None
        self.addr = None
        self._views = None
        self.n_a = self.n_o = self.min_new = None
        self.px_meta = self.blk_meta = None
        self.label_n = self.mix = self.flags = None
        self.anchor_f32 = self.contrast_f32 = None
        self.la = self.lc = None
        self.row_range = None
        self.row_ref = self.inv_norm = None
        self.max_label = 20
        self.l_po = None
        self.bf16_feats = False

    @property
    def n_c(self):
        return self.n_a + self.n_o

    def _view(self, name):
        if self._views is None:
            self._views = payload_views(self.payload, self.max_tiles, self.kpad)
        return self._views[name]

    counts = property(lambda self: self._view("counts"))
    tile_range = property(lambda self: self._view("range"))
    lab_tiles = property(lambda self: self._view("lab"))
    prob_tiles = property(lambda self: self._view("prob"))
    feat_tiles = property(lambda self: self._view("feat"))


_PINNED = {}


def _pinned_counts(dev):
    key = (dev.type, dev.index)
    buf = _PINNED.get(key)
    if buf is None:
        buf = _PINNED[key] = torch.empty(4, dtype=torch.int32).pin_memory()
    return buf


def _multi_rank():
    import torch.distributed as dist
    return dist.is_available() and dist.is_initialized() and dist.get_world_size() > 1


def _build_pack(f_n, f_o, l_po, labels, max_label, sync=True, require_new_class=True):
    _need_cuda(f_n, f_o, l_po, labels)
    if f_n.dim() != 4 or f_n.shape[1] != FEAT_DIM or f_o.shape != f_n.shape:
        raise ValueError("pre_contrastive_pixel: f_n / f_o must be [B,%d,h,w]" % FEAT_DIM)
    B, _, h, w = f_n.shape
    if l_po.dim() != 4 or l_po.shape[0] != B or tuple(l_po.shape[2:]) != (h, w):
        raise ValueError("pre_contrastive_pixel: l_po must be [B,C_old,h,w]")
    if labels.dim() != 3 or labels.shape[0] != B:
        raise ValueError("pre_contrastive_pixel: l_n must be [B,H,W]")
    L = _lib.lib()
    dev = f_n.device
    labels = labels.to(torch.int64).contiguous()
    bf16_feats = f_n.dtype == torch.bfloat16 and f_o.dtype == torch.bfloat16
    if bf16_feats:
        f_n, f_o = f_n.contiguous(), f_o.contiguous()
    else:
        f_n, f_o = _f32c(f_n), _f32c(f_o)
    l_po = _f32c(l_po)
    H, W = labels.shape[-2:]
    pk = ContrastPack()
    pk.bf16_feats = bf16_feats
    pk.shape, pk.n_px, pk.c_old = (B, h, w), B * h * w, l_po.shape[1]
    pk.kpad = L.ucd_con_prob_kpad(pk.c_old)
    pk.max_tiles = L.ucd_con_max_tiles(pk.n_px)
    n_px = pk.n_px
    i32 = dict(device=dev, dtype=torch.int32)
    pk.max_label = int(max_label)
    nb = L.ucd_con_num_bins(pk.max_label, pk.c_old)
    pk.px_meta = torch.empty(7, n_px, **i32)
    pk.label_n, pk.mix, pk.flags = pk.px_meta[0], pk.px_meta[1], pk.px_meta[2]
    pk.blk_meta = torch.empty(L.ucd_con_blk_meta_ints(n_px, nb), **i32)
    lay = payload_layout(pk.max_tiles, pk.kpad)
    pk.payload = torch.empty(lay["nbytes"], device=dev, dtype=torch.uint8)
    base = pk.payload.data_ptr()
    ad = pk.addr = {k: base + lay[k] for k in ("counts", "range", "lab", "prob", "feat")}
    st = cur_stream()
    counts_host = _pinned_counts(dev)
    check(L.ucd_con_prep_labels(ptr(labels), ptr(l_po), B, pk.c_old, h, w, H, W, pk.max_label, ptr(pk.px_meta),
                                ptr(pk.blk_meta), ad["counts"], counts_host.data_ptr(), st), "con_prep_labels")
    copied = None
    if sync:
        copied = torch.cuda.Event()
        copied.record()
    pk.anchor_f32 = torch.empty(n_px, FEAT_DIM, device=dev, dtype=torch.float32)
    pk.contrast_f32 = torch.empty(2 * n_px, FEAT_DIM, device=dev, dtype=torch.float32)
    ldt = _label_dtype(max(pk.max_label, pk.c_old - 1))
    pk.la = torch.empty(n_px, device=dev, dtype=ldt)
    pk.lc = torch.empty(2 * n_px, device=dev, dtype=ldt)
    pk.row_range = torch.empty((n_px + TILE - 1) // TILE, 2, **i32)
    pk.row_ref = torch.empty(n_px, **i32)
    pk.inv_norm = torch.empty(n_px, device=dev, dtype=torch.float32)
    pack_fn = L.ucd_con_prep_pack_bf16 if bf16_feats else L.ucd_con_prep_pack
    check(pack_fn(ptr(f_n), ptr(f_o), ptr(l_po), ptr(pk.px_meta), ptr(pk.blk_meta), ad["counts"], B,
                  pk.c_old, h, w, pk.max_label, ptr(pk.anchor_f32), ptr(pk.contrast_f32), ptr(pk.la),
                  ptr(pk.lc), pk.la.element_size(), ad["feat"], ad["prob"], ad["lab"],
                  ad["range"], ptr(pk.row_range), ptr(pk.row_ref), ptr(pk.inv_norm),
                  pk.max_tiles, st),
          "con_prep_pack")
    pk.l_po = l_po
    if not sync:
        return pk
    copied.synchronize()
    pk.n_a, pk.n_o, pk.min_new, _ = (int(v) for v in counts_host.tolist())
    if require_new_class and pk.n_a > 0 and pk.min_new > max(int(max_label), 0):
        raise RuntimeError("pre_contrastive_pixel: no new-class pixel in the batch "
                           "(the reference raises here too, utils/loss.py:355)")
    return pk


class _AnchorFn(torch.autograd.Function):

    @staticmethod
    def forward(ctx, f_n, pack):
        ctx.pack = pack
        ctx.in_dtype = f_n.dtype
        return pack.anchor_f32[:pack.n_a]

    @staticmethod
    def backward(ctx, g):
        pk = ctx.pack
        B, h, w = pk.shape
        g = _f32c(g)
        if pk.n_a == 0:
            return torch.zeros(B, FEAT_DIM, h, w, device=g.device, dtype=ctx.in_dtype), None
        direct_bf16 = pk.bf16_feats and ctx.in_dtype == torch.bfloat16
        df = torch.empty(B, FEAT_DIM, h, w, device=g.device, dtype=torch.bfloat16 if direct_bf16 else torch.float32)
        bwd_fn = _lib.lib().ucd_con_prep_bwd_bf16 if direct_bf16 else _lib.lib().ucd_con_prep_bwd
        check(bwd_fn(ptr(g), ptr(pk.anchor_f32), ptr(pk.inv_norm), ptr(pk.px_meta),
                     ptr(pk.blk_meta), ptr(df), B, h, w, cur_stream()), "con_prep_bwd")
        return df.to(ctx.in_dtype), None


class JointProb:

    def __init__(self, pack):
        self.pack = pack

    @property
    def shape(self):
        return (self.pack.n_a, self.pack.n_c)

    def dense(self):
        pk = self.pack
        B, h, w = pk.shape
        p = torch.softmax(pk.l_po.permute(0, 2, 3, 1).reshape(pk.n_px, pk.c_old), dim=1)
        anchor = (pk.flags & 1).bool()
        pseudo = (pk.flags & 2).bool()
        pa = p[anchor]
        pc = torch.cat([pa, p[pseudo]])
        P = pa @ pc.T
        la, lc = pk.la[:pk.n_a].to(torch.int32), pk.lc[:pk.n_c].to(torch.int32)
        P[(la >= pk.min_new)[:, None] & (lc >= pk.min_new)[None, :]] = 1.0
        return P

    def detach(self):
        return self


def _label_dtype(max_label):
    return torch.int8 if max_label <= 127 else torch.int32


class _RowsFn(torch.autograd.Function):

    @staticmethod
    def forward(ctx, f):
        x = _f32c(f)
        B, D, h, w = x.shape
        rows = torch.empty(B * h * w, D, device=x.device, dtype=torch.float32)
        inv = torch.empty(B * h * w, device=x.device, dtype=torch.float32)
        check(_lib.lib().ucd_rows_normalize_fwd(ptr(x), ptr(rows), ptr(inv), B, h, w, cur_stream()), "rows_normalize_fwd")
        ctx.save_for_backward(rows, inv)
        ctx.shape, ctx.in_dtype = (B, D, h, w), f.dtype
        return rows

    @staticmethod
    def backward(ctx, g):
        rows, inv = ctx.saved_tensors
        B, D, h, w = ctx.shape
        df = torch.empty(B, D, h, w, device=g.device, dtype=torch.float32)
        check(_lib.lib().ucd_rows_normalize_bwd(ptr(_f32c(g)), ptr(rows), ptr(inv), ptr(df), B, h, w, cur_stream()),
              "rows_normalize_bwd")
        return df.to(ctx.in_dtype)


def _pixel_to_pixel(f_n, l_n, f_o, max_label):
    _need_cuda(f_n, l_n, f_o)
    if f_n.dim() != 4 or f_n.shape[1] != FEAT_DIM or (f_o is not None and f_o.shape != f_n.shape):
        raise ValueError("pre_contrastive_pixel: f_n / f_o must be [B,%d,h,w]" % FEAT_DIM)
    B, _, h, w = f_n.shape
    if l_n.dim() != 3 or l_n.shape[0] != B:
        raise ValueError("pre_contrastive_pixel: l_n must be [B,H,W]")
    L = _lib.lib()
    dev = f_n.device
    labels = l_n.to(torch.int64).contiguous()
    H, W = labels.shape[-2:]
    n_px = B * h * w
    i32 = dict(device=dev, dtype=torch.int32)
    px_meta = torch.empty(7, n_px, **i32)
    blk_meta = torch.empty(L.ucd_con_blk_meta_ints(n_px, L.ucd_con_num_bins(int(max_label), 1)), **i32)
    counts = torch.empty(4, **i32)
    dummy = torch.zeros(B, 1, h, w, device=dev, dtype=torch.float32)
    check(L.ucd_con_prep_labels(ptr(labels), ptr(dummy), B, 1, h, w, H, W, int(max_label), ptr(px_meta), ptr(blk_meta),
                                ptr(counts), None, cur_stream()), "con_prep_labels")
    lab = px_meta[0].to(_label_dtype(int(max_label)))
    out = _RowsFn.apply(f_n)
    if f_o is not None:
        out = torch.cat((out, _RowsFn.apply(f_o.detach())), dim=0)
        lab = torch.cat((lab, lab))
    return out.unsqueeze(1), lab


def pre_contrastive_pixel(f_n, l_n, l_po=None, f_o=None, max_label=20, require_new_class=None):
    if l_po is None:
        return _pixel_to_pixel(f_n, l_n, f_o, max_label)
    if f_o is None:
        raise UnboundLocalError("pre_contrastive_pixel: l_po without f_o is undefined in the reference too "
                                "(utils/loss.py:399 returns an unassigned `Output`)")
    if require_new_class is None:
        require_new_class = not _multi_rank()
    pack = _build_pack(f_n.detach(), f_o.detach(), l_po.detach(), l_n, max_label, require_new_class=require_new_class)
    anchor = _AnchorFn.apply(f_n, pack)
    anchor._ucd_pack = pack
    out = (anchor, pack.contrast_f32[:pack.n_c], pack.la[:pack.n_a], pack.lc[:pack.n_c], JointProb(pack))
    return out


pre_contractive_pixel = pre_contrastive_pixel


def _local_cols(pack):
    ad = pack.addr
    return dict(feat=ad["feat"], prob=ad["prob"], lab=ad["lab"], range=ad["range"],
                counts=ad["counts"], n_chunks=1, chunk_tiles=pack.max_tiles, kpad=pack.kpad, min_new=ad["counts"] + 8,
                payload=pack.payload)


def gather_contrast_columns(payload, max_tiles, kpad, group, async_op=False):
    import torch.distributed as dist
    world, rank = dist.get_world_size(group), dist.get_rank(group)
    payload = payload.contiguous()
    buf = torch.empty(world, payload.numel(), device=payload.device, dtype=torch.uint8)
    work = dist.all_gather_into_tensor(buf.view(-1), payload, group=group, async_op=async_op)
    out = payload_views(buf, max_tiles, kpad)
    out.update(buf=buf, n_chunks=world, chunk_tiles=max_tiles, chunk_stride=payload.numel(),
               self_tile0=rank * max_tiles, rank=rank, work=work if async_op else None)
    return out


class _ConFn(torch.autograd.Function):
    @staticmethod
    def forward(ctx, anchor, cols, rows, inv_tau, p_mode, dense_p, group, ddp_scale):
        L = _lib.lib()
        dev = anchor.device
        max_row_tiles = rows["max_tiles"]
        plan_tiles = rows.get("plan_tiles", 0)
        out = torch.empty(3, device=dev, dtype=torch.float32)
        need_grad = bool(ctx.needs_input_grad[0])
        grad_unit = (torch.empty(max_row_tiles * TILE, FEAT_DIM, device=dev, dtype=torch.float32)
                     if need_grad else None)

        def run(c, part, n_chunks, stride, local_chunk, self_tile0, ws, ws_bytes):
            check(L.ucd_con_fwd(ptr(c["feat"]), ptr(c["prob"]), ptr(c["lab"]), ptr(c["counts"]), n_chunks,
                                c["chunk_tiles"], stride, local_chunk, part, ptr(rows["feat"]), ptr(rows["prob"]),
                                ptr(rows["lab"]), ptr(rows["n_rows"]), ptr(c["range"]), ptr(rows["range"]),
                                self_tile0, ptr(c["min_new"]), p_mode, c["kpad"], ptr(dense_p),
                                0 if dense_p is None else dense_p.shape[1], inv_tau, 1 if need_grad else 0, ptr(out),
                                ptr(grad_unit), ptr(ws), ws_bytes, max_row_tiles, plan_tiles, cur_stream()),
                  "con_fwd")

        if group is None:
            ws_bytes = L.ucd_con_workspace_bytes(max_row_tiles, cols["n_chunks"] * cols["chunk_tiles"], plan_tiles, 0)
            ws = torch.empty(ws_bytes, device=dev, dtype=torch.uint8)
            run(cols, 0, cols["n_chunks"], 0, -1, rows["self_tile0"], ws, ws_bytes)
        else:
            g = gather_contrast_columns(cols["payload"], cols["chunk_tiles"], cols["kpad"], group, async_op=True)
            world, rank, T = g["n_chunks"], g["rank"], cols["chunk_tiles"]
            ws_bytes = L.ucd_con_workspace_bytes(max_row_tiles, world * T, plan_tiles, T)
            ws = torch.empty(ws_bytes, device=dev, dtype=torch.uint8)
            run(cols, 1, world, g["chunk_stride"], rank, g["self_tile0"], ws, ws_bytes)
            g["work"].wait()
            gc = dict(feat=g["feat"][0], prob=g["prob"][0], lab=g["lab"][0], range=g["range"][0],
                      counts=g["counts"][0], min_new=g["counts"][0, 2:3], chunk_tiles=T, kpad=cols["kpad"])
            run(gc, 2, world, g["chunk_stride"], rank, g["self_tile0"], ws, ws_bytes)
            ctx.gathered = g["buf"]
        world = 1
        if group is not None:
            import torch.distributed as dist
            dist.all_reduce(out[:2], group=group)
            world = dist.get_world_size(group)
        n_rows = rows["n_rows"]
        if isinstance(n_rows, int):
            ctx.n_rows_addr, ctx.keep = n_rows, rows.get("keep")
            ctx.save_for_backward(grad_unit, out, None, rows.get("row_ref"))
        else:
            ctx.n_rows_addr = None
            ctx.save_for_backward(grad_unit, out, n_rows, rows.get("row_ref"))
        ctx.static_pack = rows.get("static_pack")
        ctx.n_a = anchor.shape[0] if ctx.static_pack is None else ctx.static_pack.n_px
        ctx.in_dtype = anchor.dtype
        ctx.world = world if ddp_scale else 1
        if group is not None:
            return out[0] / out[1]
        return out[2]

    @staticmethod
    def backward(ctx, g):
        grad_unit, out, n_rows, row_ref = ctx.saved_tensors
        if ctx.n_rows_addr is not None:
            n_rows = ctx.n_rows_addr
        d_anchor = torch.empty(ctx.n_a, FEAT_DIM, device=g.device, dtype=torch.float32)
        if ctx.n_a == 0:
            return d_anchor.to(ctx.in_dtype), None, None, None, None, None, None, None
        check(_lib.lib().ucd_con_bwd(ptr(grad_unit), ptr(out), ptr(_f32c(g.reshape(1))), float(ctx.world),
                                     ptr(n_rows), ptr(row_ref), ptr(d_anchor), ctx.n_a, cur_stream()), "con_bwd")
        pk = ctx.static_pack
        if pk is not None:
            B, h, w = pk.shape
            direct_bf16 = pk.bf16_feats and ctx.in_dtype == torch.bfloat16
            df = torch.empty(B, FEAT_DIM, h, w, device=g.device,
                             dtype=torch.bfloat16 if direct_bf16 else torch.float32)
            bwd_fn = _lib.lib().ucd_con_prep_bwd_bf16 if direct_bf16 else _lib.lib().ucd_con_prep_bwd
            check(bwd_fn(ptr(d_anchor), ptr(pk.anchor_f32), ptr(pk.inv_norm), ptr(pk.px_meta),
                         ptr(pk.blk_meta), ptr(df), B, h, w, cur_stream()), "con_prep_bwd")
            d_anchor = df.to(ctx.in_dtype)
        return d_anchor, None, None, None, None, None, None, None


class PixelConLossV2(nn.Module):

    def __init__(self, sample_method='none', temperature=0.07, *, gather_negatives=False, process_group=None,
                 ddp_grad_scale=True):
        super(PixelConLossV2, self).__init__()
        self.temperature = temperature
        self.sample_method = sample_method
        self.gather_negatives = gather_negatives
        self.process_group = process_group
        self.ddp_grad_scale = ddp_grad_scale
        self.max_dense_bytes = 2 << 30
        print(temperature)

    def _group(self):
        if not self.gather_negatives:
            return None
        import torch.distributed as dist
        if not (dist.is_available() and dist.is_initialized()):
            return None
        g = self.process_group if self.process_group is not None else dist.group.WORLD
        return g if dist.get_world_size(g) > 1 else None

    def forward(self, anchor_features, contrast_feature, anchor_labels, contrast_labels, P=None):
        _need_cuda(anchor_features, contrast_feature)
        inv_tau = 1.0 / float(self.temperature)
        L = _lib.lib()
        dev = anchor_features.device
        pack = P.pack if isinstance(P, JointProb) else None
        own = pack is not None and (getattr(anchor_features, "_ucd_pack", None) is pack or (
            anchor_features.dtype == torch.float32 and tuple(anchor_features.shape) == (pack.n_a, FEAT_DIM)
            and (pack.n_a == 0 or anchor_features.data_ptr() == pack.anchor_f32.data_ptr())))
        if pack is not None and not own:
            import warnings
            n_bytes = 4.0 * pack.n_a * pack.n_c
            msg = ("PixelConLossV2: anchor_features is not the tensor pre_contrastive_pixel returned (cast / clone / "
                   "slice?): falling back to a dense %d x %d joint-probability matrix (%.2f GB).  Pass the tuple "
                   "through unchanged, or use PixelContrastiveDistillation." % (pack.n_a, pack.n_c, n_bytes / 1e9))
            if n_bytes > self.max_dense_bytes:
                raise RuntimeError(msg + "  Refusing: above max_dense_bytes=%d." % self.max_dense_bytes)
            warnings.warn(msg, RuntimeWarning, stacklevel=2)
            P, pack = P.dense(), None
        if pack is not None:
            group = self._group()
            ad = pack.addr
            rows = dict(feat=ad["feat"], prob=ad["prob"], lab=ad["lab"], n_rows=ad["counts"], keep=pack.payload,
                        range=pack.row_range, row_ref=pack.row_ref, max_tiles=max(1, (pack.n_a + TILE - 1) // TILE),
                        self_tile0=0)
            cols = _local_cols(pack)
            if pack.n_a == 0 and group is None:
                return anchor_features.sum() * 0.0
            return _ConFn.apply(anchor_features, cols, rows, inv_tau, 1, None, group, self.ddp_grad_scale)

        if anchor_features.dim() != 2 or anchor_features.shape[1] != FEAT_DIM or contrast_feature.shape[1] != FEAT_DIM:
            raise ValueError("PixelConLossV2: features must be [N,%d]" % FEAT_DIM)
        n_a, n_c = anchor_features.shape[0], contrast_feature.shape[0]
        if n_a == 0 or n_c == 0:
            return anchor_features.sum() * 0.0
        if contrast_feature.requires_grad and torch.is_grad_enabled():
            raise RuntimeError("PixelConLossV2: contrast_feature requires grad, but this implementation only "
                               "differentiates w.r.t. anchor_features (the UCD prep detaches the contrast side, "
                               "utils/loss.py:366); pass contrast_feature.detach() if that is what you mean")
        a32, c32 = _f32c(anchor_features.detach()), _f32c(contrast_feature.detach())
        la = anchor_labels.reshape(-1).to(device=dev, dtype=torch.int32).contiguous()
        lc = contrast_labels.reshape(-1).to(device=dev, dtype=torch.int32).contiguous()
        if la.numel() != n_a or lc.numel() != n_c:
            raise ValueError("PixelConLossV2: label / feature counts disagree")
        rt, ct = (n_a + TILE - 1) // TILE, (n_c + TILE - 1) // TILE
        bf = dict(device=dev, dtype=torch.bfloat16)
        rfeat = torch.empty(rt, FEAT_DIM // 8, TILE, 8, **bf)
        cfeat = torch.empty(ct, FEAT_DIM // 8, TILE, 8, **bf)
        rlab = torch.empty(rt, TILE, device=dev, dtype=torch.int32)
        clab = torch.empty(ct, TILE, device=dev, dtype=torch.int32)
        st = cur_stream()
        check(L.ucd_con_pack_rows(ptr(a32), ptr(la), n_a, ptr(rfeat), ptr(rlab), rt, st), "con_pack_rows")
        check(L.ucd_con_pack_rows(ptr(c32), ptr(lc), n_c, ptr(cfeat), ptr(clab), ct, st), "con_pack_rows")
        rrange = torch.empty(rt, 2, device=dev, dtype=torch.int32)
        crange = torch.empty(ct, 2, device=dev, dtype=torch.int32)
        check(L.ucd_con_tile_ranges(ptr(rlab), rt, None, ptr(rrange), st), "con_tile_ranges")
        check(L.ucd_con_tile_ranges(ptr(clab), ct, None, ptr(crange), st), "con_tile_ranges")
        counts = torch.tensor([[n_c, 0]], device=dev, dtype=torch.int32)
        n_rows = torch.tensor([n_a], device=dev, dtype=torch.int32)
        dense_p, p_mode = None, 0
        if P is not None:
            if tuple(P.shape) != (n_a, n_c):
                raise ValueError("PixelConLossV2: P must be [N_a, N_c]")
            dense_p, p_mode = _f32c(P.detach()), 2
        cols = dict(feat=cfeat, prob=None, lab=clab, range=crange, counts=counts, n_chunks=1, chunk_tiles=ct, kpad=16,
                    min_new=None)
        rows = dict(feat=rfeat, prob=None, lab=rlab, range=rrange, n_rows=n_rows, max_tiles=rt, self_tile0=0)
        return _ConFn.apply(anchor_features, cols, rows, inv_tau, p_mode, dense_p, None, False)


class _SelfConFn(torch.autograd.Function):
    @staticmethod
    def forward(ctx, rows, labels, mode, n_anchor, inv_tau, kappa):
        L = _lib.lib()
        dev = rows.device
        n, D = rows.shape
        x = _f32c(rows.detach())
        if D < FEAT_DIM:
            x = torch.nn.functional.pad(x, (0, FEAT_DIM - D))
        lab = labels.to(device=dev, dtype=torch.int32).contiguous()
        tiles = (n + TILE - 1) // TILE
        feat = torch.empty(tiles, FEAT_DIM // 8, TILE, 8, device=dev, dtype=torch.bfloat16)
        ltile = torch.empty(tiles, TILE, device=dev, dtype=torch.int32)
        rng = torch.empty(tiles, 2, device=dev, dtype=torch.int32)
        st = cur_stream()
        check(L.ucd_con_pack_rows(ptr(x), ptr(lab), n, ptr(feat), ptr(ltile), tiles, st), "con_pack_rows")
        check(L.ucd_con_tile_ranges(ptr(ltile), tiles, None, ptr(rng), st), "con_tile_ranges")
        meta = torch.tensor([n, 0, n], device=dev, dtype=torch.int32)
        need_grad = bool(ctx.needs_input_grad[0])
        out = torch.empty(3, device=dev, dtype=torch.float32)
        grad_unit = torch.empty(n, FEAT_DIM, device=dev, dtype=torch.float32) if need_grad else None
        ws_bytes = L.ucd_selfcon_workspace_bytes(tiles)
        ws = torch.empty(ws_bytes, device=dev, dtype=torch.uint8)
        check(L.ucd_selfcon_fwd(ptr(feat), ptr(ltile), ptr(rng), ptr(meta), meta.data_ptr() + 8, n, n_anchor, mode,
                                inv_tau, kappa, 1 if need_grad else 0, ptr(out), ptr(grad_unit), ptr(ws), ws_bytes, st),
              "selfcon_fwd")
        ctx.save_for_backward(grad_unit, out, meta)
        ctx.shape, ctx.in_dtype = (n, D), rows.dtype
        return out[2]

    @staticmethod
    def backward(ctx, g):
        grad_unit, out, meta = ctx.saved_tensors
        n, D = ctx.shape
        d = torch.empty(n, FEAT_DIM, device=g.device, dtype=torch.float32)
        check(_lib.lib().ucd_con_bwd(ptr(grad_unit), ptr(out), ptr(_f32c(g.reshape(1))), 1.0, meta.data_ptr() + 8, None,
                                     ptr(d), n, cur_stream()), "con_bwd")
        return d[:, :D].to(ctx.in_dtype), None, None, None, None, None


def _selfcon_rows(features, what):
    if features.dim() < 3:
        raise ValueError('`features` needs to be [bsz, n_views, ...],'
                         'at least 3 dimensions are required')
    _need_cuda(features)
    feats = features.reshape(features.shape[0], features.shape[1], -1)
    if feats.shape[2] > FEAT_DIM:
        raise NotImplementedError("%s: feature width %d > %d is not supported by the sweep kernels"
                                  % (what, feats.shape[2], FEAT_DIM))
    return feats, feats.transpose(0, 1).reshape(-1, feats.shape[2])


class PixelConLoss(nn.Module):

    def __init__(self, sample_method='none', temperature=1):
        super().__init__()
        self.temperature = temperature
        self.sample_method = sample_method

    def forward(self, features, labels=None):
        feats, rows = _selfcon_rows(features, "PixelConLoss")
        if labels is None:
            raise AttributeError("PixelConLoss: labels are required (the reference calls labels.view, loss_new.py:376)")
        lab = labels.reshape(-1)
        if lab.numel() != feats.shape[0] or feats.shape[1] != 1:
            raise ValueError("PixelConLoss: expected features [n, 1, D] and n labels")
        lab = lab.to(rows.device)
        lab = lab - lab.min()
        return _SelfConFn.apply(rows, lab, 0, rows.shape[0], 1.0 / float(self.temperature), 1.0)


class SupConLoss(nn.Module):

    def __init__(self, temperature=0.07, contrast_mode='all', base_temperature=0.07):
        super().__init__()
        self.temperature = temperature
        self.contrast_mode = contrast_mode
        self.base_temperature = base_temperature

    def forward(self, features, labels=None, mask=None):
        feats, rows = _selfcon_rows(features, "SupConLoss")
        bsz, n_views = feats.shape[0], feats.shape[1]
        if labels is not None and mask is not None:
            raise ValueError('Cannot define both `labels` and `mask`')
        if mask is not None:
            raise NotImplementedError("SupConLoss: an explicit `mask` is not supported; pass labels (or nothing: SimCLR)")
        if labels is None:
            lab = torch.arange(bsz, device=rows.device)
        else:
            lab = labels.contiguous().view(-1).to(rows.device)
            if lab.shape[0] != bsz:
                raise ValueError('Num of labels does not match num of features')
            lab = lab - lab.min()
        if self.contrast_mode == 'one':
            n_anchor = bsz
        elif self.contrast_mode == 'all':
            n_anchor = bsz * n_views
        else:
            raise ValueError('Unknown mode: {}'.format(self.contrast_mode))
        return _SelfConFn.apply(rows, lab.repeat(n_views), 1, n_anchor, 1.0 / float(self.temperature),
                                float(self.temperature) / float(self.base_temperature))


class PixelContrastiveDistillation(nn.Module):

    def __init__(self, temperature=0.07, max_label=20, *, gather_negatives=False, process_group=None,
                 ddp_grad_scale=True, expected_anchor_fraction=1.0):
        super().__init__()
        self.temperature = temperature
        self.max_label = int(max_label)
        self.gather_negatives = gather_negatives
        self.process_group = process_group
        self.ddp_grad_scale = ddp_grad_scale
        self.expected_anchor_fraction = float(expected_anchor_fraction)

    def _group(self):
        if not self.gather_negatives:
            return None
        import torch.distributed as dist
        if not (dist.is_available() and dist.is_initialized()):
            return None
        group = self.process_group if self.process_group is not None else dist.group.WORLD
        return group if dist.get_world_size(group) > 1 else None

    def forward(self, f_n, l_n, l_po, f_o):
        pack = _build_pack(f_n.detach(), f_o.detach(), l_po.detach(), l_n, self.max_label, sync=False)
        cap_tiles = (pack.n_px + TILE - 1) // TILE
        plan_tiles = max(1, min(cap_tiles, int(cap_tiles * self.expected_anchor_fraction + 0.999)))
        ad = pack.addr
        rows = dict(feat=ad["feat"], prob=ad["prob"], lab=ad["lab"], n_rows=ad["counts"], keep=pack.payload,
                    range=pack.row_range, row_ref=pack.row_ref, max_tiles=cap_tiles, self_tile0=0,
                    plan_tiles=plan_tiles, static_pack=pack)
        group = self._group()
        cols = _local_cols(pack)
        return _ConFn.apply(f_n, cols, rows, 1.0 / float(self.temperature), 1, None, group, self.ddp_grad_scale)


class _SegFusedFn(torch.autograd.Function):
    @staticmethod
    def forward(ctx, lr, lr_old, labels, old_cl, ignore_index, alpha):
        _need_cuda(lr, lr_old, labels)
        x, t = _f32c(lr), _f32c(lr_old)
        B, C, h, w = x.shape
        C_old = t.shape[1]
        H, W = labels.shape[-2:]
        dev = x.device
        need_grad = bool(ctx.needs_input_grad[0])
        sums = torch.empty(3, device=dev, dtype=torch.float32)
        g = torch.empty(2, B, C, h, w, device=dev, dtype=torch.float32) if need_grad else None
        n_ws = int(_lib.lib().ucd_seg_fused_workspace_floats(B, C, C_old, h, w, H, W))
        if n_ws == 0:
            raise ValueError("FusedUnbiasedLosses: shapes not supported (%s)" % ((B, C, C_old, h, w, H, W),))
        ws = torch.empty(n_ws, device=dev, dtype=torch.float32)
        check(_lib.lib().ucd_seg_fused_fwd(ptr(x), ptr(t), ptr(labels), ptr(g[0]) if need_grad else None,
                                           ptr(g[1]) if need_grad else None, ptr(sums), ptr(ws), n_ws, B, C, C_old,
                                           h, w, H, W, old_cl, ignore_index, float(alpha), 1 if need_grad else 0,
                                           cur_stream()), "seg_fused_fwd")
        ctx.save_for_backward(g)
        ctx.n_px = float(B * H * W)
        ctx.in_dtype = lr.dtype
        return sums[0] / ctx.n_px, sums[2] / ctx.n_px, sums[1]

    @staticmethod
    def backward(ctx, g_ce, g_kd, _g_cnt):
        (g,) = ctx.saved_tensors
        d = g[0] * (g_ce / ctx.n_px) + g[1] * (g_kd / ctx.n_px)
        return d.to(ctx.in_dtype), None, None, None, None, None


class FusedUnbiasedLosses(nn.Module):

    def __init__(self, old_cl, ignore_index=255, alpha=1., ce_reduction='mean'):
        super().__init__()
        self.old_cl, self.ignore_index, self.alpha, self.ce_reduction = int(old_cl), int(ignore_index), alpha, ce_reduction

    def forward(self, logits_lr, logits_old_lr, labels):
        if labels.dtype != torch.int64 or labels.dim() != 3:
            raise TypeError("FusedUnbiasedLosses: labels must be int64 [B,H,W]")
        if logits_lr.dim() != 4 or logits_old_lr.dim() != 4 or logits_lr.shape[0] != labels.shape[0] \
                or logits_lr.shape[2:] != logits_old_lr.shape[2:] or logits_old_lr.shape[1] > logits_lr.shape[1]:
            raise ValueError("FusedUnbiasedLosses: logits [B,C,h,w] / old logits [B,C_old,h,w] / labels [B,H,W] disagree")
        tgt = labels if labels.is_contiguous() else labels.contiguous()
        ce, kd, cnt = _SegFusedFn.apply(logits_lr, logits_old_lr.detach(), tgt, self.old_cl, self.ignore_index, self.alpha)
        if tgt is not labels:
            labels.copy_(tgt)
        if self.ce_reduction == 'valid':
            ce = ce * (float(labels.numel()) / cnt)
        return ce, kd
```

Measured before the change: 557,900.

## Fuse CE+KD backward with bilinear upsample adjoint into low-res gradient kernel

Adds a kernel that computes the combined unbiased CE and KD pixel gradients at full resolution and immediately folds them through the bilinear-upsample adjoint, writing the gradient of the low-resolution logits directly. The Python autograd path detects when the loss input came from the package's upsample and routes the gradient to its source, skipping the full-resolution dx tensor and the separate upsample backward. This removes a large full-resolution write and re-read. In exchange it needs shape constraints, uses shared-memory staging and atomics at tile boundaries, and adds fragile autograd graph introspection.

```diff
diff --git a/include/ucd_b200.h b/include/ucd_b200.h
--- a/include/ucd_b200.h
+++ b/include/ucd_b200.h
@@ -59,6 +59,12 @@
                               void* stream);
 int ucd_upsample_bilinear_bwd(const float* gout, float* gin, int64_t planes, int h, int w, int H, int W,
                               void* stream);
+int ucd_unce_unkd_bwd_lowres(const float* x, const int64_t* y, const float* lse_all, const float* bkg_gap,
+                             const float* ce_g_px, const float* ce_g_scalar, float ce_g_mul, const float* ce_stats,
+                             int mean_over_valid, int old_cl, int ignore_index, const float* t, const float* mask,
+                             float alpha, const float* lse3, const float* kd_g_px, const float* kd_g_scalar,
+                             float kd_g_mul, int kd_variant, float* d_lr, int B, int C, int C_old, int h, int w, int H,
+                             int W, void* stream);
 
 size_t ucd_seg_fused_workspace_floats(int B, int C, int C_old, int h, int w, int H, int W);
 int ucd_seg_fused_fwd(const float* lr, const float* lr_old, int64_t* labels, float* g_ce, float* g_kd,
diff --git a/ucd_b200/_lib.py b/ucd_b200/_lib.py
--- a/ucd_b200/_lib.py
+++ b/ucd_b200/_lib.py
@@ -6,6 +6,8 @@
 LIB_PATH = os.path.join(_HERE, "libucd_b200.so")
 
 _lib = None
+
+UCD_ENOSUP = -3
 
 P = c_void_p
 _PROTOS = {
@@ -21,6 +23,8 @@
     "ucd_kd_bwd": (c_int, [P, P, P, c_float, P, P, P, c_float, P, c_int, c_int, c_int, c_int, c_int64, c_int, P]),
     "ucd_unce_unkd_bwd": (c_int, [P, P, P, P, P, P, c_float, P, c_int, c_int, c_int, P, P, c_float, P, P, P, c_float, c_int,
                                   P, c_int, c_int, c_int, c_int, c_int64, P]),
+    "ucd_unce_unkd_bwd_lowres": (c_int, [P, P, P, P, P, P, c_float, P, c_int, c_int, c_int, P, P, c_float, P, P, P,
+                                         c_float, c_int, P, c_int, c_int, c_int, c_int, c_int, c_int, c_int, P]),
     "ucd_bkg_mask": (c_int, [P, P, P, c_int, c_int, c_int64, c_int, P]),
     "ucd_upsample_bilinear_fwd": (c_int, [P, P, c_int64, c_int, c_int, c_int, c_int, P]),
     "ucd_upsample_bilinear_bwd": (c_int, [P, P, c_int64, c_int, c_int, c_int, c_int, P]),
diff --git a/ucd_b200/csrc/ce_kd.cu b/ucd_b200/csrc/ce_kd.cu
--- a/ucd_b200/csrc/ce_kd.cu
+++ b/ucd_b200/csrc/ce_kd.cu
@@ -1,4 +1,7 @@
 #include "common.cuh"
+#include "sweep_adjoint.cuh"
+
+#include <stdlib.h>
 
 namespace ucd {
 
@@ -478,6 +481,85 @@
   }
 }
 
+struct PairArgs {
+  const long long* y;
+  const float *lse_all, *bkg_gap, *ce_g_px, *t, *mask, *lse3, *kd_g_px;
+  long long plane;
+  float gs_ce, gs_kd, a2, inv_cold;
+  int old_cl, ignore_index, C, C_old, mask_zero;
+};
+
+__device__ __forceinline__ PairArgs pair_args(const long long* y, const float* lse_all, const float* bkg_gap,
+                                              const float* ce_g_px, const float* ce_g_scalar, float ce_g_mul,
+                                              const float* ce_stats, int mean_over_valid, int old_cl, int ignore_index,
+                                              const float* t, const float* mask, float alpha, const float* lse3,
+                                              const float* kd_g_px, const float* kd_g_scalar, float kd_g_mul,
+                                              int mask_zero, int B, int C, int C_old, long long HW) {
+  PairArgs a;
+  a.y = y, a.lse_all = lse_all, a.bkg_gap = bkg_gap, a.ce_g_px = ce_g_px, a.t = t, a.mask = mask, a.lse3 = lse3;
+  a.kd_g_px = kd_g_px;
+  a.plane = (long long)B * HW;
+  a.a2 = alpha * kLog2e;
+  a.inv_cold = 1.f / (float)C_old;
+  a.gs_ce = 0.f;
+  if (ce_g_px == nullptr) {
+    a.gs_ce = ce_g_scalar[0] * ce_g_mul;
+    if (mean_over_valid) a.gs_ce = a.gs_ce / ce_stats[1];
+  }
+  a.gs_kd = (kd_g_px == nullptr) ? kd_g_scalar[0] * kd_g_mul : 0.f;
+  a.old_cl = old_cl, a.ignore_index = ignore_index, a.C = C, a.C_old = C_old, a.mask_zero = mask_zero;
+  return a;
+}
+
+template <int VEC>
+struct PairCoef {
+  float la2[VEC], lt2[VEC], uce[VEC], ukd[VEC], fold[VEC], fb[VEC];
+  int lab[VEC];
+};
+
+template <int VEC>
+__device__ __forceinline__ void pair_coef(const PairArgs& a, long long px, const float* tp, PairCoef<VEC>& q) {
+  float la[VEC], lo[VEC], lb[VEC], lt[VEC], gp[VEC], gk[VEC], mk[VEC], u0[VEC];
+  Vec<VEC>::load_cached(a.lse_all + px, la);
+  Vec<VEC>::load_cached(a.bkg_gap + px, lo);
+  Vec<VEC>::load_cached(a.lse3 + a.plane + px, lb);
+  Vec<VEC>::load_cached(a.lse3 + 2 * a.plane + px, lt);
+  Vec<VEC>::load_cached(tp, u0);
+  if (a.ce_g_px != nullptr) Vec<VEC>::load_cached(a.ce_g_px + px, gp);
+  if (a.kd_g_px != nullptr) Vec<VEC>::load_cached(a.kd_g_px + px, gk);
+  if (a.mask != nullptr) Vec<VEC>::load_cached(a.mask + px, mk);
+  const long long* yp = a.y + px;
+#pragma unroll
+  for (int i = 0; i < VEC; ++i) {
+    long long tt = yp[i];
+    if (tt < a.old_cl) tt = 0;
+    const bool dead = (tt == a.ignore_index) || tt < 0 || tt >= a.C;
+    q.lab[i] = dead ? -1 : (int)tt;
+    q.uce[i] = dead ? 0.f : (a.ce_g_px != nullptr ? gp[i] : a.gs_ce);
+    q.la2[i] = la[i] * kLog2e;
+    q.lt2[i] = lt[i] * kLog2e;
+    q.fold[i] = ex2f(lo[i] * kLog2e);
+    float u = (a.kd_g_px != nullptr ? gk[i] : a.gs_kd) * a.inv_cold;
+    if (a.mask != nullptr) u *= a.mask_zero ? (mk[i] == 0.f ? 1.f : 0.f) : mk[i];
+    q.ukd[i] = u;
+    const float q0 = ex2f(fmaf(u0[i], a.a2, -q.lt2[i]));
+    q.fb[i] = q0 * ex2f((la[i] - lb[i]) * kLog2e);
+  }
+}
+
+template <int VEC>
+__device__ __forceinline__ float pair_dx(const PairArgs& a, const PairCoef<VEC>& q, int i, int c, bool old_fg, float v,
+                                         float u) {
+  const float pr = ex2f(fmaf(v, kLog2e, -q.la2[i]));
+  float sub_ce;
+  if (q.lab[i] == 0 && a.old_cl > 0)
+    sub_ce = (c < a.old_cl) ? pr * q.fold[i] : 0.f;
+  else
+    sub_ce = (c == q.lab[i]) ? 1.f : 0.f;
+  const float sub_kd = old_fg ? ex2f(fmaf(u, a.a2, -q.lt2[i])) : pr * q.fb[i];
+  return fmaf(q.uce[i], pr - sub_ce, q.ukd[i] * (pr - sub_kd));
+}
+
 template <int VEC, bool ACC>
 __global__ void __launch_bounds__(kStreamThreads)
 unce_unkd_bwd_kernel(const float* __restrict__ x, const long long* __restrict__ y, const float* __restrict__ lse_all,
@@ -489,51 +571,17 @@
                      int mask_zero, float* __restrict__ dx, int B, int C, int C_old, long long HW) {
   const long long gpi = HW / VEC;
   const long long n_groups = gpi * B;
-  const long long plane = (long long)B * HW;
-  const float a2 = alpha * kLog2e;
-  const float inv_cold = 1.f / (float)C_old;
-  float gs_ce = 0.f;
-  if (ce_g_px == nullptr) {
-    gs_ce = ce_g_scalar[0] * ce_g_mul;
-    if (mean_over_valid) gs_ce = gs_ce / ce_stats[1];
-  }
-  const float gs_kd = (kd_g_px == nullptr) ? kd_g_scalar[0] * kd_g_mul : 0.f;
+  const PairArgs a = pair_args(y, lse_all, bkg_gap, ce_g_px, ce_g_scalar, ce_g_mul, ce_stats, mean_over_valid, old_cl,
+                               ignore_index, t, mask, alpha, lse3, kd_g_px, kd_g_scalar, kd_g_mul, mask_zero, B, C,
+                               C_old, HW);
   for (long long g = (long long)blockIdx.x * blockDim.x + threadIdx.x; g < n_groups;
        g += (long long)gridDim.x * blockDim.x) {
     const long long b = g / gpi, p = (g - b * gpi) * VEC;
     const float* xp = x + (b * C) * HW + p;
     const float* tp = t + (b * C_old) * HW + p;
     float* dp = dx + (b * C) * HW + p;
-    const long long* yp = y + b * HW + p;
-    float la2[VEC], lt2[VEC], uce[VEC], ukd[VEC], fold[VEC], fb[VEC];
-    int lab[VEC];
-    {
-      float la[VEC], lo[VEC], lb[VEC], lt[VEC], gp[VEC], gk[VEC], mk[VEC], u0[VEC];
-      Vec<VEC>::load_cached(lse_all + b * HW + p, la);
-      Vec<VEC>::load_cached(bkg_gap + b * HW + p, lo);
-      Vec<VEC>::load_cached(lse3 + plane + b * HW + p, lb);
-      Vec<VEC>::load_cached(lse3 + 2 * plane + b * HW + p, lt);
-      Vec<VEC>::load_cached(tp, u0);
-      if (ce_g_px != nullptr) Vec<VEC>::load_cached(ce_g_px + b * HW + p, gp);
-      if (kd_g_px != nullptr) Vec<VEC>::load_cached(kd_g_px + b * HW + p, gk);
-      if (mask != nullptr) Vec<VEC>::load_cached(mask + b * HW + p, mk);
-#pragma unroll
-      for (int i = 0; i < VEC; ++i) {
-        long long tt = yp[i];
-        if (tt < old_cl) tt = 0;
-        const bool dead = (tt == ignore_index) || tt < 0 || tt >= C;
-        lab[i] = dead ? -1 : (int)tt;
-        uce[i] = dead ? 0.f : (ce_g_px != nullptr ? gp[i] : gs_ce);
-        la2[i] = la[i] * kLog2e;
-        lt2[i] = lt[i] * kLog2e;
-        fold[i] = ex2f(lo[i] * kLog2e);
-        float u = (kd_g_px != nullptr ? gk[i] : gs_kd) * inv_cold;
-        if (mask != nullptr) u *= mask_zero ? (mk[i] == 0.f ? 1.f : 0.f) : mk[i];
-        ukd[i] = u;
-        const float q0 = ex2f(fmaf(u0[i], a2, -lt2[i]));
-        fb[i] = q0 * ex2f((la[i] - lb[i]) * kLog2e);
-      }
-    }
+    PairCoef<VEC> q;
+    pair_coef<VEC>(a, b * HW + p, tp, q);
 #pragma unroll 4
     for (int c = 0; c < C; ++c) {
       float v[VEC], u[VEC], o[VEC];
@@ -541,17 +589,122 @@
       const bool old_fg = c >= 1 && c < C_old;
       if (old_fg) Vec<VEC>::load(tp + (long long)c * HW, u);
 #pragma unroll
-      for (int i = 0; i < VEC; ++i) {
-        const float pr = ex2f(fmaf(v[i], kLog2e, -la2[i]));
-        float sub_ce;
-        if (lab[i] == 0 && old_cl > 0)
-          sub_ce = (c < old_cl) ? pr * fold[i] : 0.f;
-        else
-          sub_ce = (c == lab[i]) ? 1.f : 0.f;
-        const float sub_kd = old_fg ? ex2f(fmaf(u[i], a2, -lt2[i])) : pr * fb[i];
-        o[i] = fmaf(uce[i], pr - sub_ce, ukd[i] * (pr - sub_kd));
-      }
+      for (int i = 0; i < VEC; ++i) o[i] = pair_dx<VEC>(a, q, i, c, old_fg, v[i], u[i]);
       store_dx<VEC, ACC>(dp + (long long)c * HW, o);
+    }
+  }
+}
+
+template <int KMAX, int NREG>
+__global__ void __maxnreg__(NREG)
+unce_unkd_bwd_lowres_kernel(const float* __restrict__ x, const long long* __restrict__ y,
+                            const float* __restrict__ lse_all, const float* __restrict__ bkg_gap,
+                            const float* __restrict__ ce_g_px, const float* __restrict__ ce_g_scalar, float ce_g_mul,
+                            const float* __restrict__ ce_stats, int mean_over_valid, int old_cl, int ignore_index,
+                            const float* __restrict__ t, const float* __restrict__ mask, float alpha,
+                            const float* __restrict__ lse3, const float* __restrict__ kd_g_px,
+                            const float* __restrict__ kd_g_scalar, float kd_g_mul, int mask_zero,
+                            float* __restrict__ d_lr, int B, int C, int C_old, int h, int w, int H, int W,
+                            float scale_h, float scale_w, int n_ranges, int range_rows, int n_cgroups, int ny_cap) {
+  extern __shared__ __align__(16) uint8_t lr_dyn[];
+  const int wv = blockDim.x;
+  const int tid = threadIdx.x;
+  float2* s_p = reinterpret_cast<float2*>(lr_dyn);
+  short4* s_j = reinterpret_cast<short4*>(s_p + 2 * KMAX * wv);
+  float2* s_h = reinterpret_cast<float2*>(s_j + w);
+  int* s_k = reinterpret_cast<int*>(s_h + ny_cap);
+  int* s_x0 = s_k + ny_cap;
+  int* s_x1 = s_x0 + wv;
+  __shared__ int s_lim[2];
+  const long long HW = (long long)H * W;
+  const PairArgs a = pair_args(y, lse_all, bkg_gap, ce_g_px, ce_g_scalar, ce_g_mul, ce_stats, mean_over_valid, old_cl,
+                               ignore_index, t, mask, alpha, lse3, kd_g_px, kd_g_scalar, kd_g_mul, mask_zero, B, C,
+                               C_old, HW);
+  const int cg = blockIdx.x % n_cgroups;
+  const int rest = blockIdx.x / n_cgroups;
+  const int rg = rest % n_ranges;
+  const long long b = rest / n_ranges;
+  const int c0 = (int)((long long)cg * C / n_cgroups), kc = (int)((long long)(cg + 1) * C / n_cgroups) - c0;
+  const int y0 = rg * range_rows, ylast = min(h, y0 + range_rows) - 1;
+  float wx0[4], wx1[4];
+  sweep_x_taps(tid, wv, w, W, scale_w, wx0, wx1, s_x0, s_x1, s_j);
+  int i_lo, i_hi;
+  const int Ylo = sweep_y_taps(tid, wv, y0, ylast, h, H, scale_h, ny_cap, s_k, s_h, s_lim, i_lo, i_hi);
+  const int X = tid * 4;
+  const float* xb = x + (b * C + c0) * HW + X;
+  const float* tb = t + b * C_old * HW + X;
+  float* out = d_lr + (b * C + c0) * (long long)h * w;
+  float2 a0[KMAX], a1[KMAX];
+#pragma unroll
+  for (int j = 0; j < KMAX; ++j) a0[j] = a1[j] = make_float2(0.f, 0.f);
+  int cur = -1, flip = 0;
+  auto emit = [&](int row, bool shared) {
+    float2* sp = s_p + flip * KMAX * wv;
+#pragma unroll
+    for (int j = 0; j < KMAX; ++j)
+      if (j < kc) sp[j * wv + tid] = a0[j];
+    __syncthreads();
+    for (int o = tid; o < kc * w; o += wv) {
+      const int j = o / w, xo = o - j * w;
+      const short4 jr = s_j[xo];
+      const float2* pj = sp + j * wv;
+      float acc = 0.f;
+      for (int i = jr.x; i < jr.y; ++i) acc += pj[i].x;
+      for (int i = jr.z; i < jr.w; ++i) acc += pj[i].y;
+      float* dst = out + ((long long)j * h + row) * w + xo;
+      if (shared)
+        atomicAdd(dst, acc);
+      else
+        *dst = acc;
+    }
+    flip ^= 1;
+  };
+#pragma unroll 1
+  for (int i = i_lo; i < i_hi; ++i) {
+    const int k = s_k[i];
+    if (k != cur) {
+      if (cur >= 0) {
+        emit(cur, cur == y0 && y0 > 0);
+#pragma unroll
+        for (int j = 0; j < KMAX; ++j) a0[j] = a1[j], a1[j] = make_float2(0.f, 0.f);
+      }
+      cur = k;
+    }
+    const long long row = (long long)(Ylo + i) * W;
+    PairCoef<4> q;
+    pair_coef<4>(a, b * HW + row + X, tb + row, q);
+    const float2 hw = s_h[i];
+#pragma unroll
+    for (int j0 = 0; j0 < KMAX; j0 += 4) {
+      float v[4][4], u[4][4];
+#pragma unroll
+      for (int jj = 0; jj < 4; ++jj) {
+        const int c = c0 + j0 + jj;
+        if (j0 + jj < kc) Vec<4>::load(xb + (long long)(j0 + jj) * HW + row, v[jj]);
+        if (j0 + jj < kc && c >= 1 && c < C_old) Vec<4>::load(tb + (long long)c * HW + row, u[jj]);
+      }
+#pragma unroll
+      for (int jj = 0; jj < 4; ++jj) {
+        const int j = j0 + jj, c = c0 + j;
+        if (j < kc) {
+          const bool old_fg = c >= 1 && c < C_old;
+          float o[4];
+#pragma unroll
+          for (int e = 0; e < 4; ++e) o[e] = pair_dx<4>(a, q, e, c, old_fg, v[jj][e], u[jj][e]);
+          const float p0 = fmaf(o[3], wx0[3], fmaf(o[2], wx0[2], fmaf(o[1], wx0[1], o[0] * wx0[0])));
+          const float p1 = fmaf(o[3], wx1[3], fmaf(o[2], wx1[2], fmaf(o[1], wx1[1], o[0] * wx1[0])));
+          a0[j].x = fmaf(hw.x, p0, a0[j].x), a0[j].y = fmaf(hw.x, p1, a0[j].y);
+          a1[j].x = fmaf(hw.y, p0, a1[j].x), a1[j].y = fmaf(hw.y, p1, a1[j].y);
+        }
+      }
+    }
+  }
+  if (cur >= 0) {
+    emit(cur, cur == y0 && y0 > 0);
+    if (ylast < h - 1) {
+#pragma unroll
+      for (int j = 0; j < KMAX; ++j) a0[j] = a1[j];
+      emit(ylast + 1, true);
     }
   }
 }
@@ -733,3 +886,84 @@
   UCD_CHECK_LAUNCH("unce_unkd_bwd_kernel");
   return UCD_OK;
 }
+
+extern "C" int ucd_unce_unkd_bwd_lowres(const float* x, const int64_t* y, const float* lse_all, const float* bkg_gap,
+                                        const float* ce_g_px, const float* ce_g_scalar, float ce_g_mul,
+                                        const float* ce_stats, int mean_over_valid, int old_cl, int ignore_index,
+                                        const float* t, const float* mask, float alpha, const float* lse3,
+                                        const float* kd_g_px, const float* kd_g_scalar, float kd_g_mul, int kd_variant,
+                                        float* d_lr, int B, int C, int C_old, int h, int w, int H, int W,
+                                        void* stream) {
+  UCD_CHECK_ARG(x && y && lse_all && bkg_gap && t && lse3 && d_lr, "ucd_unce_unkd_bwd_lowres: null pointer");
+  UCD_CHECK_ARG((ce_g_px || ce_g_scalar) && (kd_g_px || kd_g_scalar),
+                "ucd_unce_unkd_bwd_lowres: need g_px or g_scalar for both terms");
+  UCD_CHECK_ARG(!mean_over_valid || ce_stats, "ucd_unce_unkd_bwd_lowres: mean_over_valid needs stats");
+  UCD_CHECK_ARG(B > 0 && C_old >= 1 && C >= C_old && h > 0 && w > 0 && H > 0 && W > 0,
+                "ucd_unce_unkd_bwd_lowres: bad shape");
+  UCD_CHECK_ARG(kd_variant == 0 || kd_variant == 2,
+                "ucd_unce_unkd_bwd_lowres: KD variant must be 0 (unbiased) or 2 (masked)");
+  const int up = H / h;
+  const bool ok = H % h == 0 && W % w == 0 && (W / w) % 8 == 0 && W / 4 <= 256 && (W / 4) % 32 == 0 && w <= W / 4 &&
+                  can_vec4((long long)H * W, {x, lse_all, bkg_gap, ce_g_px, t, mask, lse3, kd_g_px}) && aligned16(y) &&
+                  up <= 64;
+  if (!ok) {
+    set_error("ucd_unce_unkd_bwd_lowres: %dx%d -> %dx%d is not a sweep-form shape", h, w, H, W);
+    return UCD_ENOSUP;
+  }
+  cudaStream_t st = (cudaStream_t)stream;
+  const int wv = W / 4;
+  struct Variant {
+    int k, nreg;
+    void (*fn)(const float*, const long long*, const float*, const float*, const float*, const float*, float,
+               const float*, int, int, int, const float*, const float*, float, const float*, const float*,
+               const float*, float, int, float*, int, int, int, int, int, int, int, float, float, int, int, int, int);
+  };
+  static const Variant variants[] = {{8, 128, unce_unkd_bwd_lowres_kernel<8, 128>},
+                                     {4, 128, unce_unkd_bwd_lowres_kernel<4, 128>},
+#ifdef UCD_DEBUG_KNOBS
+                                     {4, 96, unce_unkd_bwd_lowres_kernel<4, 96>},
+                                     {8, 112, unce_unkd_bwd_lowres_kernel<8, 112>},
+#endif
+  };
+  int vi = 0;
+#ifdef UCD_DEBUG_KNOBS
+  if (const char* e = getenv("UCD_LRB_VARIANT")) vi = (atoi(e) >= 0 && atoi(e) < 4) ? atoi(e) : 0;
+#endif
+  const Variant& var = variants[vi];
+  const int min_groups = (C + var.k - 1) / var.k;
+  int groups = min_groups, rows = h;
+  const long long want = 2ll * kNumSMs * (65536 / var.nreg / 32 * 32);
+  auto threads = [&](int r, int g) { return (long long)B * ((h + r - 1) / r) * g * wv; };
+  while (rows > 1 && threads(rows, groups) < want) rows = (rows + 1) / 2;
+  while (groups < C && threads(rows, groups) < want) ++groups;
+  auto dyn_bytes = [&](int r) {
+    return (size_t)2 * var.k * wv * 8 + (size_t)w * 8 + (size_t)((r + 2) * up + 8) * 12 + (size_t)2 * wv * 4;
+  };
+#ifdef UCD_DEBUG_KNOBS
+  if (const char* e = getenv("UCD_LRB_ROWS")) rows = atoi(e) > 0 ? min(atoi(e), h) : rows;
+  if (const char* e = getenv("UCD_LRB_GROUPS")) groups = atoi(e) >= min_groups ? min(atoi(e), C) : groups;
+#endif
+  while (rows > 1 && dyn_bytes(rows) > 200 * 1024) rows = (rows + 1) / 2;
+  const int n_ranges = (h + rows - 1) / rows;
+  const long long nb = (long long)B * n_ranges * groups;
+  if (nb >= (1ll << 31) || dyn_bytes(rows) > 200 * 1024) {
+    set_error("ucd_unce_unkd_bwd_lowres: B=%d h=%d H=%d needs more blocks or shared memory than one launch has", B, h, H);
+    return UCD_ENOSUP;
+  }
+  const int ny_cap = (rows + 2) * up + 8;
+  const size_t dyn = dyn_bytes(rows);
+  auto kern = var.fn;
+  cudaError_t e;
+  if (dyn > 48 * 1024) {
+    e = cudaFuncSetAttribute(kern, cudaFuncAttributeMaxDynamicSharedMemorySize, (int)dyn);
+    if (e != cudaSuccess) return cuda_fail(e, "cudaFuncSetAttribute(unce_unkd_bwd_lowres)");
+  }
+  e = cudaMemsetAsync(d_lr, 0, (size_t)B * C * h * w * sizeof(float), st);
+  if (e != cudaSuccess) return cuda_fail(e, "cudaMemsetAsync(unce_unkd_bwd_lowres)");
+  kern<<<(unsigned)nb, wv, dyn, st>>>(x, (const long long*)y, lse_all, bkg_gap, ce_g_px, ce_g_scalar, ce_g_mul,
+                                      ce_stats, mean_over_valid, old_cl, ignore_index, t, mask, alpha, lse3, kd_g_px,
+                                      kd_g_scalar, kd_g_mul, kd_variant == 2 ? 1 : 0, d_lr, B, C, C_old, h, w, H, W,
+                                      (float)h / (float)H, (float)w / (float)W, n_ranges, rows, groups, ny_cap);
+  UCD_CHECK_LAUNCH("unce_unkd_bwd_lowres_kernel");
+  return UCD_OK;
+}
diff --git a/ucd_b200/csrc/sweep_adjoint.cuh b/ucd_b200/csrc/sweep_adjoint.cuh
--- /dev/null
+++ b/ucd_b200/csrc/sweep_adjoint.cuh
@@ -0,0 +1,64 @@
+#pragma once
+#include "common.cuh"
+
+namespace ucd {
+
+__device__ __forceinline__ void sweep_x_taps(int tid, int wv, int w, int W, float scale_w, float (&wx0)[4],
+                                             float (&wx1)[4], int* s_x0, int* s_x1, short4* s_j) {
+  const int X = tid * 4;
+  {
+    const Tap t0 = bilinear_tap(X, scale_w, w, W);
+    s_x0[tid] = t0.i0, s_x1[tid] = t0.i1;
+#pragma unroll
+    for (int i = 0; i < 4; ++i) {
+      const Tap tx = bilinear_tap(X + i, scale_w, w, W);
+      wx0[i] = tx.w0, wx1[i] = tx.w1;
+    }
+  }
+  __syncthreads();
+  if (tid < w) {
+    const int sc4 = (W / w) / 4;
+    const int j0 = max((tid - 2) * sc4 - 2, 0), j1 = min((tid + 2) * sc4 + 2, wv - 1);
+    int a0 = 0, a1 = 0, b0 = 0, b1 = 0;
+    bool fa = false, fb = false;
+    for (int j = j0; j <= j1; ++j) {
+      if (s_x0[j] == tid) {
+        if (!fa) a0 = j, fa = true;
+        a1 = j + 1;
+      }
+      if (s_x1[j] == tid) {
+        if (!fb) b0 = j, fb = true;
+        b1 = j + 1;
+      }
+    }
+    s_j[tid] = make_short4((short)a0, (short)a1, (short)b0, (short)b1);
+  }
+}
+
+__device__ __forceinline__ int sweep_y_taps(int tid, int nthr, int y0, int ylast, int h, int H, float scale_h, int ny_cap,
+                                            int* s_k, float2* s_h, int* s_lim, int& i_lo, int& i_hi) {
+  const float inv = (float)H / (float)h;
+  int Ylo = (int)floorf(((float)y0 - 0.5f) * inv) - 2, Yhi = (int)ceilf(((float)ylast + 1.5f) * inv) + 2;
+  Ylo = max(Ylo, 0), Yhi = min(Yhi, H - 1);
+  const int ny = min(Yhi - Ylo + 1, ny_cap);
+  __syncthreads();
+  for (int i = tid; i < ny; i += nthr) {
+    const Tap ty = bilinear_tap(Ylo + i, scale_h, h, H);
+    s_k[i] = ty.i0;
+    const bool clamped = ty.i1 == ty.i0;
+    s_h[i] = make_float2(clamped ? ty.w0 + ty.w1 : ty.w0, clamped ? 0.f : ty.w1);
+  }
+  __syncthreads();
+  for (int i = tid; i < ny; i += nthr) {
+    const int k = s_k[i];
+    if (k >= y0 && k <= ylast) {
+      if (i == 0 || s_k[i - 1] < y0) s_lim[0] = i;
+      if (i == ny - 1 || s_k[i + 1] > ylast) s_lim[1] = i + 1;
+    }
+  }
+  __syncthreads();
+  i_lo = s_lim[0], i_hi = s_lim[1];
+  return Ylo;
+}
+
+}
diff --git a/ucd_b200/csrc/upsample.cu b/ucd_b200/csrc/upsample.cu
--- a/ucd_b200/csrc/upsample.cu
+++ b/ucd_b200/csrc/upsample.cu
@@ -1,4 +1,5 @@
 #include "common.cuh"
+#include "sweep_adjoint.cuh"
 
 #include <stdlib.h>
 
@@ -261,42 +262,15 @@
   const int tid = threadIdx.x;
   float4* ring = reinterpret_cast<float4*>(up_dyn);
   float2* s_p = reinterpret_cast<float2*>(ring + (size_t)UN * wv);
-  float2* s_h = s_p + 2 * wv;
+  short4* s_j = reinterpret_cast<short4*>(s_p + 2 * wv);
+  float2* s_h = reinterpret_cast<float2*>(s_j + w);
   int* s_k = reinterpret_cast<int*>(s_h + ny_cap);
   int* s_x0 = s_k + ny_cap;
   int* s_x1 = s_x0 + wv;
-  short4* s_j = reinterpret_cast<short4*>(s_x1 + wv);
   __shared__ int s_lim[2];
   const int X = tid * 4;
   float wx0[4], wx1[4];
-  {
-    const Tap t0 = bilinear_tap(X, scale_w, w, W);
-    s_x0[tid] = t0.i0, s_x1[tid] = t0.i1;
-#pragma unroll
-    for (int i = 0; i < 4; ++i) {
-      const Tap tx = bilinear_tap(X + i, scale_w, w, W);
-      wx0[i] = tx.w0, wx1[i] = tx.w1;
-    }
-  }
-  __syncthreads();
-  if (tid < w) {
-    const int sc4 = (W / w) / 4;
-    const int j0 = max((tid - 2) * sc4 - 2, 0), j1 = min((tid + 2) * sc4 + 2, wv - 1);
-    int a0 = 0, a1 = 0, b0 = 0, b1 = 0;
-    bool fa = false, fb = false;
-    for (int j = j0; j <= j1; ++j) {
-      if (s_x0[j] == tid) {
-        if (!fa) a0 = j, fa = true;
-        a1 = j + 1;
-      }
-      if (s_x1[j] == tid) {
-        if (!fb) b0 = j, fb = true;
-        b1 = j + 1;
-      }
-    }
-    s_j[tid] = make_short4((short)a0, (short)a1, (short)b0, (short)b1);
-  }
-  const float inv = (float)H / (float)h;
+  sweep_x_taps(tid, wv, w, W, scale_w, wx0, wx1, s_x0, s_x1, s_j);
   const uint32_t ring_s = (uint32_t)__cvta_generic_to_shared(ring + tid);
   const uint32_t slot_b = (uint32_t)wv * 16u;
   int flip = 0;
@@ -307,26 +281,8 @@
     const int y0 = (int)(r - plane * h);
     const int ylast = (int)min((long long)min(h, y0 + cap_rows), y0 + (r_end - r)) - 1;
     r += ylast - y0 + 1;
-    int Ylo = (int)floorf(((float)y0 - 0.5f) * inv) - 2, Yhi = (int)ceilf(((float)ylast + 1.5f) * inv) + 2;
-    Ylo = max(Ylo, 0), Yhi = min(Yhi, H - 1);
-    const int ny = min(Yhi - Ylo + 1, ny_cap);
-    __syncthreads();
-    for (int i = tid; i < ny; i += wv) {
-      const Tap ty = bilinear_tap(Ylo + i, scale_h, h, H);
-      s_k[i] = ty.i0;
-      const bool clamped = ty.i1 == ty.i0;
-      s_h[i] = make_float2(clamped ? ty.w0 + ty.w1 : ty.w0, clamped ? 0.f : ty.w1);
-    }
-    __syncthreads();
-    for (int i = tid; i < ny; i += wv) {
-      const int k = s_k[i];
-      if (k >= y0 && k <= ylast) {
-        if (i == 0 || s_k[i - 1] < y0) s_lim[0] = i;
-        if (i == ny - 1 || s_k[i + 1] > ylast) s_lim[1] = i + 1;
-      }
-    }
-    __syncthreads();
-    const int i_lo = s_lim[0], i_hi = s_lim[1];
+    int i_lo, i_hi;
+    const int Ylo = sweep_y_taps(tid, wv, y0, ylast, h, H, scale_h, ny_cap, s_k, s_h, s_lim, i_lo, i_hi);
     const float* gp = gout + (size_t)plane * H * W + (size_t)(Ylo + i_lo) * W + X;
     float* out = gin + (size_t)plane * h * w;
     float a0p0 = 0.f, a0p1 = 0.f, a1p0 = 0.f, a1p1 = 0.f, c0 = 0.f, c1 = 0.f;
diff --git a/ucd_b200/losses.py b/ucd_b200/losses.py
--- a/ucd_b200/losses.py
+++ b/ucd_b200/losses.py
@@ -1,4 +1,6 @@
 from __future__ import annotations
+
+import weakref
 
 import torch
 import torch.nn as nn
@@ -42,6 +44,7 @@
     @staticmethod
     def forward(ctx, x, out_h, out_w):
         _need_cuda(x)
+        ctx.set_materialize_grads(False)
         x = _f32c(x)
         lead, (h, w) = x.shape[:-2], x.shape[-2:]
         planes = 1
@@ -56,6 +59,8 @@
 
     @staticmethod
     def backward(ctx, g):
+        if g is None:
+            return None, None, None
         lead, h, w, out_h, out_w, planes = ctx.shape
         g = _f32c(g)
         gin = torch.empty(*lead, h, w, device=g.device, dtype=torch.float32)
@@ -66,7 +71,43 @@
 
 
 def interpolate_bilinear(x, size):
-    return _UpsampleFn.apply(x, int(size[0]), int(size[1]))
+    out = _UpsampleFn.apply(x, int(size[0]), int(size[1]))
+    if out.requires_grad:
+        out._ucd_upsample = (x, x._version, out._version)
+    return out
+
+
+class _Route:
+
+    __slots__ = ("lr_shape", "out_ref", "out_hw", "probe_node")
+    _probes = {}
+
+    def __init__(self, src, out, probe_node):
+        self.lr_shape, self.out_hw, self.probe_node = tuple(src.shape), tuple(out.shape[2:]), probe_node
+        self.out_ref = weakref.ref(out)
+
+    @staticmethod
+    def of(outputs):
+        rec = getattr(outputs, "_ucd_upsample", None)
+        if rec is None:
+            return None
+        src, src_version, out_version = rec
+        if (src._version != src_version or outputs._version != out_version or not src.requires_grad
+                or src.dim() != 4 or outputs.dim() != 4):
+            return None
+        probe = _Route._probes.get(outputs.device)
+        if probe is None:
+            probe = _Route._probes[outputs.device] = torch.empty((), device=outputs.device, requires_grad=True)
+        return _Route(src, outputs, torch.autograd.graph.get_gradient_edge(probe).node), src, probe
+
+    def route_now(self):
+        out = self.out_ref()
+        if out is None or out.retains_grad or out._backward_hooks:
+            return False
+        try:
+            return bool(torch._C._will_engine_execute_node(self.probe_node))
+        except Exception:
+            return False
 
 
 class _GradChain:
@@ -86,26 +127,57 @@
             chain = t._ucd_grad_chain = _GradChain()
         return chain
 
-    def submit(self, term, seq, is_head):
+    def submit(self, term, seq, is_head, route=None):
         self.closed = True
         if seq == self.calls:
             self.pending = []
         if not is_head:
             if term is not None:
                 self.pending.append(term)
-            return None, None
+            return None, None, None
         terms, self.pending = self.pending + ([term] if term is not None else []), []
         self.token = None
-        return (_launch_terms(terms) if terms else None), None
+        if not terms:
+            return None, None, None
+        d_lr = _launch_lowres(terms, route) if route is not None else None
+        if d_lr is not None:
+            return None, None, d_lr
+        return _launch_terms(terms), None, None
+
+
+def _pair(terms):
+    ce = [t for t in terms if t["kind"] == "ce"]
+    kd = [t for t in terms if t["kind"] == "kd" and t["variant"] in (0, 2)]
+    if ce and kd and ce[0]["C"] == kd[0]["C"] and ce[0]["HW"] == kd[0]["HW"]:
+        return ce[0], kd[0]
+    return None
+
+
+def _launch_lowres(terms, route):
+    pair = _pair(terms)
+    if pair is None or len(terms) != 2 or not route.route_now():
+        return None
+    c, k = pair
+    B, C, h, w = route.lr_shape
+    H, W = route.out_hw
+    d_lr = torch.empty(B, C, h, w, device=c["x"].device, dtype=torch.float32)
+    rc = _lib.lib().ucd_unce_unkd_bwd_lowres(
+        ptr(c["x"]), ptr(c["targets"]), ptr(c["lse"][0]), ptr(c["lse"][1]), ptr(c["g_px"]), ptr(c["g_sc"]), 1.0,
+        ptr(c["stats"]), c["mean_over_valid"], c["old_cl"], c["ignore_index"], ptr(k["t"]), ptr(k["m"]), k["alpha"],
+        ptr(k["lse3"]), ptr(k["g_px"]), ptr(k["g_sc"]), k["g_mul"], k["variant"], ptr(d_lr), B, C, k["C_old"], h, w,
+        H, W, cur_stream())
+    if rc == _lib.UCD_ENOSUP:
+        return None
+    check(rc, "unce_unkd_bwd_lowres")
+    return d_lr
 
 
 def _launch_terms(terms):
     dx = torch.empty_like(terms[0]["x"])
-    ce = [t for t in terms if t["kind"] == "ce"]
-    kd = [t for t in terms if t["kind"] == "kd" and t["variant"] in (0, 2)]
+    pair = _pair(terms)
     acc = False
-    if ce and kd and ce[0]["C"] == kd[0]["C"] and ce[0]["HW"] == kd[0]["HW"]:
-        c, k = ce[0], kd[0]
+    if pair is not None:
+        c, k = pair
         check(_lib.lib().ucd_unce_unkd_bwd(
             ptr(c["x"]), ptr(c["targets"]), ptr(c["lse"][0]), ptr(c["lse"][1]), ptr(c["g_px"]), ptr(c["g_sc"]), 1.0,
             ptr(c["stats"]), c["mean_over_valid"], c["old_cl"], c["ignore_index"], ptr(k["t"]), ptr(k["m"]), k["alpha"],
@@ -133,8 +205,10 @@
 
 class _UnceFn(torch.autograd.Function):
     @staticmethod
-    def forward(ctx, inputs, targets, old_cl, ignore_index, reduction, chain=None, link=None):
+    def forward(ctx, inputs, targets, old_cl, ignore_index, reduction, chain=None, link=None, route=None, src=None,
+                probe=None):
         ctx.chain, ctx.is_head, ctx.seq = chain, link is None, (chain.calls if chain is not None else 0)
+        ctx.route = route
         ctx.set_materialize_grads(False)
         B, C = inputs.shape[0], inputs.shape[1]
         HW = inputs.numel() // max(B * C, 1)
@@ -161,9 +235,9 @@
         B, C, HW, old_cl, ignore_index, reduction = ctx.cfg
         if g is None:
             if ctx.chain is None:
-                return None, None, None, None, None, None, None
-            d_in, d_link = ctx.chain.submit(None, ctx.seq, ctx.is_head)
-            return d_in, None, None, None, None, None, d_link
+                return (None,) * 10
+            d_in, d_link, d_src = ctx.chain.submit(None, ctx.seq, ctx.is_head, ctx.route)
+            return d_in, None, None, None, None, None, d_link, None, d_src, None
         g_px, g_sc = None, None
         if reduction == "none":
             g_sc = _scalar_grad(g)
@@ -179,17 +253,23 @@
         if ctx.chain is None:
             dx = torch.empty_like(x)
             _launch_term(term, dx, False)
-            return dx, None, None, None, None, None, None
-        d_in, d_link = ctx.chain.submit(term, ctx.seq, ctx.is_head)
-        return d_in, None, None, None, None, None, d_link
+            return (dx,) + (None,) * 9
+        d_in, d_link, d_src = ctx.chain.submit(term, ctx.seq, ctx.is_head, ctx.route)
+        return d_in, None, None, None, None, None, d_link, None, d_src, None
 
 
 def _chained(fn, inputs, args):
     chain = _GradChain.of(inputs)
     if chain is None:
         return fn.apply(inputs, *args)
+    route = None
+    if chain.token is None:
+        route = _Route.of(inputs)
     chain.calls += 1
-    out, token = fn.apply(inputs, *args, chain, chain.token)
+    if route is None:
+        out, token = fn.apply(inputs, *args, chain, chain.token)
+    else:
+        out, token = fn.apply(inputs, *args, chain, chain.token, *route)
     chain.token = token
     return out
 
@@ -220,8 +300,10 @@
 
 class _UnkdFn(torch.autograd.Function):
     @staticmethod
-    def forward(ctx, inputs, targets, mask, alpha, reduction, variant=0, chain=None, link=None):
+    def forward(ctx, inputs, targets, mask, alpha, reduction, variant=0, chain=None, link=None, route=None, src=None,
+                probe=None):
         ctx.chain, ctx.is_head, ctx.seq = chain, link is None, (chain.calls if chain is not None else 0)
+        ctx.route = route
         ctx.set_materialize_grads(False)
         B, C, C_old = inputs.shape[0], inputs.shape[1], targets.shape[1]
         HW = inputs.numel() // max(B * C, 1)
@@ -249,9 +331,9 @@
         B, C, C_old, HW, alpha, reduction, variant = ctx.cfg
         if g is None:
             if ctx.chain is None:
-                return None, None, None, None, None, None, None, None
-            d_in, d_link = ctx.chain.submit(None, ctx.seq, ctx.is_head)
-            return d_in, None, None, None, None, None, None, d_link
+                return (None,) * 11
+            d_in, d_link, d_src = ctx.chain.submit(None, ctx.seq, ctx.is_head, ctx.route)
+            return d_in, None, None, None, None, None, None, d_link, None, d_src, None
         g_px, g_sc, g_mul = None, None, 1.0
         if reduction == "none":
             g_sc = _scalar_grad(g)
@@ -268,9 +350,9 @@
         if ctx.chain is None:
             dx = torch.empty_like(x)
             _launch_term(term, dx, False)
-            return dx, None, None, None, None, None, None, None
-        d_in, d_link = ctx.chain.submit(term, ctx.seq, ctx.is_head)
-        return d_in, None, None, None, None, None, None, d_link
+            return (dx,) + (None,) * 10
+        d_in, d_link, d_src = ctx.chain.submit(term, ctx.seq, ctx.is_head, ctx.route)
+        return d_in, None, None, None, None, None, None, d_link, None, d_src, None
 
 
 class UnbiasedKnowledgeDistillationLoss(nn.Module):
```

Result: faster. 578,700, median of 6 (+3.7%).
